# matter-labs/era-zkevm_test_harness

Measured on AMD Instinct MI355X. Metric: base-layer circuits/sec (2^20 rows); full-block synth wall-time 1/8 GPU, higher is better.
Workload: dtype u64 (Goldilocks, p = 2^64 - 2^32 + 1)

## Files before the change

era_zkevm_test_harness_amd/csrc/radix_sort.cuh:

```cuda
#pragma once
#include "zkw_ctx.h"

namespace zkw {

constexpr int RS_ROUNDS = 8, RS_WAVES = 4, RS_TILE = RS_WAVES * RS_ROUNDS * 64, RS_CHUNK = 16384;

template <class K>
static __device__ __forceinline__ unsigned rs_digit(K key, unsigned shift, unsigned mask) { return (unsigned)(key >> shift) & mask; }

template <class K>
static __device__ __forceinline__ void k_rs_hist(const VB& vb, const K* __restrict__ keys, size_t n, unsigned shift, unsigned mask, u32* __restrict__ hist, u32 n_tiles) {
    __shared__ u32 cnt[256];
    const int t = threadIdx.x;
    cnt[t] = 0;
    __syncthreads();
    const size_t base = (size_t)vb.x * RS_TILE;
#pragma unroll 4
    for (int r = 0; r < RS_TILE / 256; r++) {
        const size_t i = base + (size_t)r * 256 + t;
        if (i < n) atomicAdd(&cnt[rs_digit(keys[i], shift, mask)], 1u);
    }
    __syncthreads();
    hist[(size_t)t * n_tiles + vb.x] = cnt[t];
}

static __device__ __forceinline__ void k_rs_scan_a(const VB& vb, u32* __restrict__ hist, size_t n_entries, u32* __restrict__ chunk_tot) {
    __shared__ u32 s_wave[16];
    const int t = threadIdx.x, lane = t & 63, wave = t >> 6;
    const size_t base = (size_t)vb.x * RS_CHUNK + (size_t)t * 16;
    u32 v[16], sum = 0;
#pragma unroll
    for (int k = 0; k < 16; k++) {
        v[k] = base + k < n_entries ? hist[base + k] : 0;
        sum += v[k];
    }
    u32 incl = sum;
#pragma unroll
    for (int off = 1; off < 64; off <<= 1) {
        const u32 y = __shfl_up(incl, off, 64);
        if (lane >= off) incl += y;
    }
    if (lane == 63) s_wave[wave] = incl;
    __syncthreads();
    u32 before = 0;
    for (int w = 0; w < wave; w++) before += s_wave[w];
    u32 run = before + incl - sum;
#pragma unroll
    for (int k = 0; k < 16; k++) {
        if (base + k < n_entries) hist[base + k] = run;
        run += v[k];
    }
    if (t == 1023) chunk_tot[vb.x] = before + incl;
}

static __device__ __forceinline__ void k_rs_scan_b(const VB& vb, u32* __restrict__ chunk_tot, u32 n_chunks) {
    __shared__ u32 s_wave[16];
    __shared__ u32 carry;
    const int t = threadIdx.x, lane = t & 63, wave = t >> 6;
    if (t == 0) carry = 0;
    __syncthreads();
    for (u32 base = 0; base < n_chunks; base += 1024) {
        const u32 i = base + t;
        const u32 v = i < n_chunks ? chunk_tot[i] : 0;
        u32 incl = v;
#pragma unroll
        for (int off = 1; off < 64; off <<= 1) {
            const u32 y = __shfl_up(incl, off, 64);
            if (lane >= off) incl += y;
        }
        if (lane == 63) s_wave[wave] = incl;
        __syncthreads();
        u32 before = carry;
        for (int w = 0; w < wave; w++) before += s_wave[w];
        if (i < n_chunks) chunk_tot[i] = before + incl - v;
        __syncthreads();
        if (t == 1023) carry = before + incl;
        __syncthreads();
    }
}

template <class K>
static __device__ __forceinline__ void k_rs_scatter(const VB& vb, const K* __restrict__ kin, const u32* __restrict__ vin, size_t n, unsigned shift, unsigned mask,
                                    const u32* __restrict__ hist, const u32* __restrict__ chunk_off, u32 n_tiles, K* __restrict__ kout, u32* __restrict__ vout) {
    __shared__ K s_key[RS_TILE];
    __shared__ u32 s_val[RS_TILE];
    __shared__ u32 wcnt[RS_WAVES][256];
    __shared__ u32 s_first[256];
    __shared__ u32 s_gbase[256];
    __shared__ u32 s_wsum[RS_WAVES];
    const int t = threadIdx.x, lane = t & 63, wave = t >> 6;
#pragma unroll
    for (int w = 0; w < RS_WAVES; w++) wcnt[w][t] = 0;
    __syncthreads();
    const size_t tile0 = (size_t)vb.x * RS_TILE, base = tile0 + (size_t)wave * (RS_ROUNDS * 64) + lane;
    K key[RS_ROUNDS];
    u32 val[RS_ROUNDS];
    unsigned long long same[RS_ROUNDS];
#pragma unroll
    for (int r = 0; r < RS_ROUNDS; r++) {
        const size_t i = base + (size_t)r * 64;
        key[r] = i < n ? kin[i] : (K)0;
        val[r] = i < n ? vin[i] : 0u;
    }
#pragma unroll
    for (int r = 0; r < RS_ROUNDS; r++) {
        const size_t i = base + (size_t)r * 64;
        const bool ok = i < n;
        const unsigned d = rs_digit(key[r], shift, mask);
        unsigned long long m = __ballot(ok);
#pragma unroll
        for (int b = 0; b < 8; b++) {
            const unsigned long long bal = __ballot((d >> b) & 1);
            m &= ((d >> b) & 1) ? bal : ~bal;
        }
        same[r] = ok ? m : 0ull;
        if (ok && (m & ((1ull << lane) - 1)) == 0) wcnt[wave][d] += (u32)__popcll(m);
        __builtin_amdgcn_wave_barrier();
    }
    __syncthreads();
    {
        u32 c[RS_WAVES], total = 0;
#pragma unroll
        for (int w = 0; w < RS_WAVES; w++) { c[w] = wcnt[w][t]; total += c[w]; }
        u32 incl = total;
#pragma unroll
        for (int off = 1; off < 64; off <<= 1) {
            const u32 y = __shfl_up(incl, off, 64);
            if (lane >= off) incl += y;
        }
        if (lane == 63) s_wsum[wave] = incl;
        __syncthreads();
        u32 first = incl - total;
        for (int w = 0; w < wave; w++) first += s_wsum[w];
        s_first[t] = first;
        const size_t e = (size_t)t * n_tiles + vb.x;
        s_gbase[t] = hist[e] + chunk_off[e / RS_CHUNK] - first;
        u32 at = first;
#pragma unroll
        for (int w = 0; w < RS_WAVES; w++) { wcnt[w][t] = at; at += c[w]; }
    }
    __syncthreads();
#pragma unroll
    for (int r = 0; r < RS_ROUNDS; r++) {
        const unsigned long long m = same[r];
        if (m) {
            const unsigned d = rs_digit(key[r], shift, mask);
            const u32 at = wcnt[wave][d] + (u32)__popcll(m & ((1ull << lane) - 1));
            s_key[at] = key[r];
            s_val[at] = val[r];
        }
        __builtin_amdgcn_wave_barrier();
        if (m && (m & ((1ull << lane) - 1)) == 0) wcnt[wave][rs_digit(key[r], shift, mask)] += (u32)__popcll(m);
        __builtin_amdgcn_wave_barrier();
    }
    __syncthreads();
    const u32 in_tile = (u32)(n - tile0 < (size_t)RS_TILE ? n - tile0 : (size_t)RS_TILE);
#pragma unroll 4
    for (u32 p = t; p < in_tile; p += 256) {
        const K k = s_key[p];
        const u32 at = s_gbase[rs_digit(k, shift, mask)] + p;
        kout[at] = k;
        vout[at] = s_val[p];
    }
}

static inline size_t rs_tiles(size_t n) { return (n + RS_TILE - 1) / RS_TILE; }
static inline size_t radix_temp_bytes(size_t n) {
    const size_t entries = 256 * rs_tiles(n), chunks = (entries + RS_CHUNK - 1) / RS_CHUNK;
    return ((n * 8 + 255) & ~(size_t)255) + ((n * 4 + 255) & ~(size_t)255) + entries * 4 + chunks * 4 + 1024;
}

template <class K>
static int radix_sort_pairs(zkw_ctx* ctx, void* tmp, size_t tmp_bytes, const K* kin, K* kout, const u32* vin, u32* vout, size_t n, unsigned end_bit) {
    if (n == 0) return ZKW_OK;
    if (n >= (1ull << 32)) return fail(ZKW_ERR_INVALID, "radix_sort_pairs: more than 2^32 - 1 pairs");
    if (tmp_bytes < radix_temp_bytes(n)) return fail(ZKW_ERR_INVALID, "radix_sort_pairs: temporary storage too small");
    if (end_bit == 0) end_bit = 1;
    const unsigned passes = (end_bit + 7) / 8;
    const u32 n_tiles = (u32)rs_tiles(n);
    const size_t entries = (size_t)256 * n_tiles;
    const u32 n_chunks = (u32)((entries + RS_CHUNK - 1) / RS_CHUNK);
    char* p = static_cast<char*>(tmp);
    K* tk = reinterpret_cast<K*>(p);
    u32* tv = reinterpret_cast<u32*>(p + ((n * 8 + 255) & ~(size_t)255));
    u32* hist = reinterpret_cast<u32*>(p + ((n * 8 + 255) & ~(size_t)255) + ((n * 4 + 255) & ~(size_t)255));
    u32* chunk = hist + entries;
    const K* src_k = kin;
    const u32* src_v = vin;
    for (unsigned pass = 0; pass < passes; pass++) {
        const bool to_out = ((passes - pass) & 1) == 1;
        K* dst_k = to_out ? kout : tk;
        u32* dst_v = to_out ? vout : tv;
        const unsigned shift = 8 * pass, bits = std::min(8u, end_bit - shift), mask = (1u << bits) - 1;
        ZKW_LAUNCH_T(ctx, (k_rs_hist<K>), "k_rs_hist", n_tiles, 256, src_k, n, shift, mask, hist, n_tiles);
        ZKW_LAUNCH(ctx, k_rs_scan_a, n_chunks, 1024, hist, entries, chunk);
        ZKW_LAUNCH(ctx, k_rs_scan_b, 1, 1024, chunk, n_chunks);
        ZKW_LAUNCH_T(ctx, (k_rs_scatter<K>), "k_rs_scatter", n_tiles, 256, src_k, src_v, n, shift, mask, (const u32*)hist, (const u32*)chunk, n_tiles, dst_k, dst_v);
        src_k = dst_k;
        src_v = dst_v;
    }
    return ZKW_OK;
}

}
```

era_zkevm_test_harness_amd/csrc/ram_kernels.cuh:

```cuda
#pragma once
#include "../../include/zkw_types.h"
#include "poseidon2.cuh"

namespace zkw {
using gl::u32;
using gl::u64;

__device__ __forceinline__ void encode_mem_query(const zkw_mem_query& q, u64 out[8]) {
    const u32* v = q.value;
    out[0] = q.timestamp;
    out[1] = q.page;
    out[2] = (u64)q.index | ((u64)(q.rw_flag ? 1 : 0) << 32) | ((u64)(q.value_is_pointer ? 1 : 0) << 33);
    u64 b5 = v[5], b6 = v[6], b7 = v[7];
    out[3] = (u64)v[0] | ((b5 & 0xFFFFFF) << 32);
    out[4] = (u64)v[1] | ((b5 >> 24) << 32) | ((b6 & 0xFFFF) << 40);
    out[5] = (u64)v[2] | ((b6 >> 16) << 32) | ((b7 & 0xFF) << 48);
    out[6] = (u64)v[3] | ((b7 >> 8) << 32);
    out[7] = v[4];
}

static __device__ __forceinline__ void k_encode_mem(const VB& vb, const zkw_mem_query* __restrict__ q, size_t n,
                                                    u64* __restrict__ enc) {
    size_t i = (size_t)vb.x * blockDim.x + threadIdx.x;
    size_t stride = (size_t)vb.nx * blockDim.x;
    for (; i < n; i += stride) {
        const uint4* src = reinterpret_cast<const uint4*>(q + i);
        uint4 w0 = src[0], w1 = src[1], w2 = src[2];
        zkw_mem_query m;
        uint4* dst = reinterpret_cast<uint4*>(&m);
        dst[0] = w0; dst[1] = w1; dst[2] = w2;
        u64 e[8];
        encode_mem_query(m, e);
        ulonglong2* o = reinterpret_cast<ulonglong2*>(enc + 8 * i);
        o[0] = make_ulonglong2(e[0], e[1]); o[1] = make_ulonglong2(e[2], e[3]);
        o[2] = make_ulonglong2(e[4], e[5]); o[3] = make_ulonglong2(e[6], e[7]);
    }
}

struct ChainJob {
    const u64* enc;
    u64* tails;
    const u64* tail_in;
    u64 n;
    u64* caps;
    u64* marks;
    u64 period;
    const zkw_mem_query* q;
    const u32* perm;
};

struct RawQuery { uint4 a, b, c; };
__device__ __forceinline__ RawQuery load_raw_query(const zkw_mem_query* q) {
    const uint4* src = reinterpret_cast<const uint4*>(q);
    RawQuery r;
    r.a = src[0]; r.b = src[1]; r.c = src[2];
    return r;
}
__device__ __forceinline__ void encode_raw_query(const RawQuery& r, u64 e[8]) {
    zkw_mem_query m;
    uint4* dm = reinterpret_cast<uint4*>(&m);
    dm[0] = r.a; dm[1] = r.b; dm[2] = r.c;
    encode_mem_query(m, e);
}
__device__ __forceinline__ u64 pick8(const u64 e[8], int g) {
    u64 v = e[0];
#pragma unroll
    for (int k = 1; k < 8; k++) v = g == k ? e[k] : v;
    return v;
}


struct RowForm {
    static constexpr int LANES = 16, N = 1, R = 1;
    p2::Coop co;
    int g;
    __device__ __forceinline__ void init(int j) { g = j; co.init(j); }
    __device__ __forceinline__ bool reads_items() const { return g < 8; }
    __device__ __forceinline__ void load_tail(const u64* t, u64 x[N]) const { x[0] = (co.active && t) ? t[g] : 0; }
    __device__ __forceinline__ void load_rate(const u64* enc, u64 e[R]) const { e[0] = enc[g]; }
    __device__ __forceinline__ void pick_rate(const u64 ew[8], u64 e[R]) const { e[0] = pick8(ew, g); }
    __device__ __forceinline__ void absorb_permute(u64 x[N], const u64 e[R]) const { x[0] = co.permute(g < 8 ? e[0] : x[0]); }
    __device__ __forceinline__ void store_tail(u64* t, const u64 p[N]) const { if (co.active) t[g] = p[0]; }
    __device__ __forceinline__ void store_caps(u64* c, const u64 p[N]) const { if (g >= 8 && g < 12) c[g - 8] = p[0]; }
};

struct QuadForm {
    static constexpr int LANES = 4, N = 3, R = 2;
    p2::Coop4 co;
    int j;
    __device__ __forceinline__ void init(int j_) { j = j_; co.init(j_); }
    __device__ __forceinline__ bool reads_items() const { return true; }
    __device__ __forceinline__ void load_tail(const u64* t, u64 x[N]) const {
#pragma unroll
        for (int c = 0; c < 3; c++) x[c] = t ? t[4 * c + j] : 0;
    }
    __device__ __forceinline__ void load_rate(const u64* enc, u64 e[R]) const { e[0] = enc[j]; e[1] = enc[4 + j]; }
    __device__ __forceinline__ void pick_rate(const u64 ew[8], u64 e[R]) const { e[0] = pick8(ew, j); e[1] = pick8(ew, 4 + j); }
    __device__ __forceinline__ void absorb_permute(u64 x[N], const u64 e[R]) const { x[0] = e[0]; x[1] = e[1]; co.permute(x); }
    __device__ __forceinline__ void store_tail(u64* t, const u64 p[N]) const {
#pragma unroll
        for (int c = 0; c < 3; c++) t[4 * c + j] = p[c];
    }
    __device__ __forceinline__ void store_caps(u64* c, const u64 p[N]) const { c[j] = p[2]; }
};

struct PairForm {
    static constexpr int LANES = 2, N = 6, R = 4;
    p2::Coop2 co;
    int j;
    __device__ __forceinline__ void init(int j_) { j = j_; co.init(j_); }
    __device__ __forceinline__ bool reads_items() const { return true; }
    __device__ __forceinline__ void load_tail(const u64* t, u64 x[N]) const {
#pragma unroll
        for (int c = 0; c < 3; c++) {
            x[2 * c] = t ? t[4 * c + 2 * j] : 0;
            x[2 * c + 1] = t ? t[4 * c + 2 * j + 1] : 0;
        }
    }
    __device__ __forceinline__ void load_rate(const u64* enc, u64 e[R]) const {
        const ulonglong2 lo = *reinterpret_cast<const ulonglong2*>(enc + 2 * j), hi = *reinterpret_cast<const ulonglong2*>(enc + 4 + 2 * j);
        e[0] = lo.x; e[1] = lo.y; e[2] = hi.x; e[3] = hi.y;
    }
    __device__ __forceinline__ void pick_rate(const u64 ew[8], u64 e[R]) const {
        e[0] = j ? ew[2] : ew[0];
        e[1] = j ? ew[3] : ew[1];
        e[2] = j ? ew[6] : ew[4];
        e[3] = j ? ew[7] : ew[5];
    }
    __device__ __forceinline__ void absorb_permute(u64 x[N], const u64 e[R]) const {
#pragma unroll
        for (int k = 0; k < 4; k++) x[k] = e[k];
        co.permute(x);
    }
    __device__ __forceinline__ void store_tail(u64* t, const u64 p[N]) const {
#pragma unroll
        for (int c = 0; c < 3; c++) *reinterpret_cast<ulonglong2*>(t + 4 * c + 2 * j) = make_ulonglong2(p[2 * c], p[2 * c + 1]);
    }
    __device__ __forceinline__ void store_caps(u64* c, const u64 p[N]) const { *reinterpret_cast<ulonglong2*>(c + 2 * j) = make_ulonglong2(p[4], p[5]); }
};

struct LaneForm {
    static constexpr int LANES = 1, N = 12, R = 8;
    __device__ __forceinline__ void init(int) {}
    __device__ __forceinline__ bool reads_items() const { return true; }
    __device__ __forceinline__ void load_tail(const u64* t, u64 x[N]) const {
#pragma unroll
        for (int k = 0; k < 12; k++) x[k] = t ? t[k] : 0;
    }
    __device__ __forceinline__ void load_rate(const u64* enc, u64 e[R]) const {
        const ulonglong2* src = reinterpret_cast<const ulonglong2*>(enc);
#pragma unroll
        for (int k = 0; k < 4; k++) { const ulonglong2 v = src[k]; e[2 * k] = v.x; e[2 * k + 1] = v.y; }
    }
    __device__ __forceinline__ void pick_rate(const u64 ew[8], u64 e[R]) const {
#pragma unroll
        for (int k = 0; k < 8; k++) e[k] = ew[k];
    }
    __device__ __forceinline__ void absorb_permute(u64 x[N], const u64 e[R]) const {
#pragma unroll
        for (int k = 0; k < 8; k++) x[k] = e[k];
        p2::permute(x);
    }
    __device__ __forceinline__ void store_tail(u64* t, const u64 p[N]) const {
        ulonglong2* d = reinterpret_cast<ulonglong2*>(t);
#pragma unroll
        for (int k = 0; k < 6; k++) d[k] = make_ulonglong2(p[2 * k], p[2 * k + 1]);
    }
    __device__ __forceinline__ void store_caps(u64* c, const u64 p[N]) const {
        ulonglong2* d = reinterpret_cast<ulonglong2*>(c);
        d[0] = make_ulonglong2(p[8], p[9]);
        d[1] = make_ulonglong2(p[10], p[11]);
    }
};

template <class Form, int WAVES>
static __device__ __forceinline__ void chain_body(const ChainJob* __restrict__ jobs, int n_jobs) {
    __builtin_amdgcn_s_setprio(3);
    const int chain = blockIdx.x * (64 * WAVES / Form::LANES) + threadIdx.x / Form::LANES;
    Form form;
    form.init(threadIdx.x % Form::LANES);
    ChainJob job;
    memset(&job, 0, sizeof job);
    if (chain < n_jobs) job = jobs[chain];
    u64 x[Form::N];
    form.load_tail(job.tail_in, x);
    const bool reads = form.reads_items();
    const bool from_q = job.enc == nullptr;
    u64 e_next[Form::R] = {};
    RawQuery rq_next;
    rq_next.a = rq_next.b = rq_next.c = make_uint4(0, 0, 0, 0);
    u64 at_next = 0;
    if (reads && job.n > 0) {
        if (from_q) rq_next = load_raw_query(job.q + (job.perm ? job.perm[0] : 0)); else form.load_rate(job.enc, e_next);
    }
    if (reads && from_q && job.n > 1) at_next = job.perm ? job.perm[1] : 1;
    u64 next_mark = job.marks ? job.period : ~0ull, mark_idx = 0;
    u64 pend[Form::N] = {}, pend_i = 0;
    bool have_pend = false, pend_mark = false;
    auto flush = [&]() {
        if (!have_pend) return;
        if (job.tails) form.store_tail(job.tails + 12 * pend_i, pend);
        if (job.caps) form.store_caps(job.caps + 4 * pend_i, pend);
        if (pend_mark) form.store_tail(job.marks + 12 * mark_idx++, pend);
        have_pend = false;
    };
    for (u64 i = 0; __any(i < job.n); i++) {
        const bool live = i < job.n;
        u64 e[Form::R];
        if (from_q) {
            u64 ew[8];
            encode_raw_query(rq_next, ew);
            form.pick_rate(ew, e);
        } else {
#pragma unroll
            for (int k = 0; k < Form::R; k++) e[k] = e_next[k];
        }
        flush();
        if (reads && i + 1 < job.n) {
            if (from_q) {
                rq_next = load_raw_query(job.q + at_next);
                if (i + 2 < job.n) at_next = job.perm ? job.perm[i + 2] : i + 2;
            } else {
                form.load_rate(job.enc + 8 * (i + 1), e_next);
            }
        }
        form.absorb_permute(x, e);
        if (live) {
#pragma unroll
            for (int k = 0; k < Form::N; k++) pend[k] = gl::canon(x[k]);
            pend_i = i;
            have_pend = true;
            pend_mark = job.marks && (i + 1 == next_mark || i + 1 == job.n);
            if (pend_mark) next_mark += job.period;
        }
    }
    flush();
}
static __global__ __launch_bounds__(64) void k_chain_full(const ChainJob* __restrict__ jobs, int n_jobs) { chain_body<RowForm, 1>(jobs, n_jobs); }
static __global__ __launch_bounds__(256) void k_chain_full_x4(const ChainJob* __restrict__ jobs, int n_jobs) { chain_body<RowForm, 4>(jobs, n_jobs); }
static __global__ __launch_bounds__(64) void k_chain_full_q4(const ChainJob* __restrict__ jobs, int n_jobs) { chain_body<QuadForm, 1>(jobs, n_jobs); }
static __global__ __launch_bounds__(256) void k_chain_full_q4x4(const ChainJob* __restrict__ jobs, int n_jobs) { chain_body<QuadForm, 4>(jobs, n_jobs); }
static __global__ __launch_bounds__(64) void k_chain_full_p2(const ChainJob* __restrict__ jobs, int n_jobs) { chain_body<PairForm, 1>(jobs, n_jobs); }
static __global__ __launch_bounds__(64) void k_chain_full_lane(const ChainJob* __restrict__ jobs, int n_jobs) { chain_body<LaneForm, 1>(jobs, n_jobs); }

struct FsJob {
    const u64* tail_u;
    const u64* tail_s;
    u32 len_u, len_s;
    u64* out;
};

static __device__ __forceinline__ void k_fs_challenges(const VB& vb, const FsJob* __restrict__ jobs, int n_jobs, int state_w, int n_chal) {
    int j = vb.x * blockDim.x + threadIdx.x;
    if (j >= n_jobs) return;
    const FsJob job = jobs[j];
    const int m = 2 * state_w + 2;
    auto elem = [&](int e) -> u64 {
        if (e >= m) return 0;
        if (e < state_w) return job.tail_u[e];
        if (e == state_w) return job.len_u;
        if (e < 2 * state_w + 1) return job.tail_s[e - state_w - 1];
        return job.len_s;
    };
    u64 s[12];
#pragma unroll
    for (int i = 0; i < 12; i++) s[i] = 0;
    s[11] = (u64)m;
    for (int i = 0; i < m; i += 8) {
#pragma unroll
        for (int k = 0; k < 8; k++) s[k] = elem(i + k);
        p2::permute(s);
    }
    int can_take = 8;
    for (int rep = 0; rep < 2; rep++) {
        job.out[rep * n_chal] = 1;
        for (int k = 1; k < n_chal; k++) {
            if (can_take == 0) { p2::permute(s); can_take = 8; }
            u64 v = 0;
#pragma unroll
            for (int q = 0; q < 8; q++) v = (q == 8 - can_take) ? s[q] : v;
            job.out[rep * n_chal + k] = gl::canon(v);
            can_take--;
        }
    }
}

constexpr int GP_BLOCK = 256;
constexpr int GP_SLABS = 4;
constexpr int GP_TILE = GP_BLOCK * GP_SLABS;

struct GpSeg {
    const u64* rows;
    u64* z;
    const u64* chal;
    u64 n;
    u32 first_tile;
    u32 n_tiles;
    const zkw_mem_query* mem_q;
    const u32* perm;
};
struct GpTile {
    u32 seg;
    u32 tile;
};

__device__ __forceinline__ u64 wave_scan_mul(u64 v, int lane) {
#pragma unroll
    for (int d = 1; d < 64; d <<= 1) {
        u64 o = __shfl_up(v, d, 64);
        if (lane >= d) v = gl::mul(v, o);
    }
    return v;
}

template <int W, int REPS>
static __device__ __forceinline__ void k_gp_local(const VB& vb, const GpSeg* __restrict__ segs,
                                                       const GpTile* __restrict__ tiles,
                                                       u64* __restrict__ tile_aggr ) {
    __shared__ u64 sh_ch[REPS][W + 1];
    __shared__ u64 sh_wave[REPS][GP_BLOCK / 64];
    const GpTile t = tiles[vb.x];
    const GpSeg seg = segs[t.seg];
    const int tid = threadIdx.x, lane = tid & 63, wave = tid >> 6;
    for (int k = tid; k < REPS * (W + 1); k += GP_BLOCK) sh_ch[k / (W + 1)][k % (W + 1)] = seg.chal[k];
    __syncthreads();
    u64 carry[REPS];
#pragma unroll
    for (int r = 0; r < REPS; r++) carry[r] = 1;
    const u64 base = (u64)t.tile * GP_TILE;
    for (int slab = 0; slab < GP_SLABS; slab++) {
        const u64 row = base + (u64)slab * GP_BLOCK + tid;
        const bool live = row < seg.n;
        u64 term[REPS];
#pragma unroll
        for (int r = 0; r < REPS; r++) term[r] = 1;
        if (live) {
            u64 e[W];
            if (W == 8 && seg.rows == nullptr) {
                u64 e8[8];
                encode_raw_query(load_raw_query(seg.mem_q + (seg.perm ? seg.perm[row] : row)), e8);
#pragma unroll
                for (int k = 0; k < (W < 8 ? W : 8); k++) e[k] = e8[k];
            } else {
                const ulonglong2* src = reinterpret_cast<const ulonglong2*>(seg.rows + row * W);
#pragma unroll
                for (int k = 0; k < W / 2; k++) { ulonglong2 w = src[k]; e[2 * k] = w.x; e[2 * k + 1] = w.y; }
            }
#pragma unroll
            for (int r = 0; r < REPS; r++) {
                u64 acc = sh_ch[r][W];
#pragma unroll
                for (int k = 0; k < W; k++) acc = gl::add(acc, gl::mul(e[k], sh_ch[r][k]));
                term[r] = acc;
            }
        }
#pragma unroll
        for (int r = 0; r < REPS; r++) {
            u64 v = wave_scan_mul(term[r], lane);
            if (lane == 63) sh_wave[r][wave] = v;
            __syncthreads();
            u64 pre = carry[r];
            for (int w = 0; w < wave; w++) pre = gl::mul(pre, sh_wave[r][w]);
            v = gl::mul(v, pre);
            if (live) seg.z[(u64)r * seg.n + row] = v;
            u64 tot = carry[r];
            for (int w = 0; w < GP_BLOCK / 64; w++) tot = gl::mul(tot, sh_wave[r][w]);
            carry[r] = tot;
            __syncthreads();
        }
    }
    if (tid == 0) {
#pragma unroll
        for (int r = 0; r < REPS; r++) tile_aggr[(u64)vb.x * REPS + r] = carry[r];
    }
}

template <int REPS>
static __device__ __forceinline__ void k_gp_tiles(const VB& vb, const GpSeg* __restrict__ segs, int n_segs, u64* __restrict__ tile_aggr) {
    int j = vb.x * blockDim.x + threadIdx.x;
    if (j >= n_segs * REPS) return;
    const GpSeg seg = segs[j / REPS];
    const int r = j % REPS;
    u64 acc = 1;
    for (u32 t = 0; t < seg.n_tiles; t++) {
        u64* p = tile_aggr + (u64)(seg.first_tile + t) * REPS + r;
        u64 v = *p;
        *p = acc;
        acc = gl::mul(acc, v);
    }
}

template <int REPS>
static __device__ __forceinline__ void k_gp_apply(const VB& vb, const GpSeg* __restrict__ segs,
                                                       const GpTile* __restrict__ tiles,
                                                       const u64* __restrict__ tile_prefix) {
    const GpTile t = tiles[vb.x];
    const GpSeg seg = segs[t.seg];
    const u64 base = (u64)t.tile * GP_TILE;
#pragma unroll
    for (int r = 0; r < REPS; r++) {
        const u64 pre = tile_prefix[(u64)vb.x * REPS + r];
        u64* z = seg.z + (u64)r * seg.n;
        for (int slab = 0; slab < GP_SLABS; slab++) {
            const u64 row = base + (u64)slab * GP_BLOCK + threadIdx.x;
            if (row < seg.n) z[row] = gl::canon(gl::mul(z[row], pre));
        }
    }
}

static __device__ __forceinline__ void k_ram_sort_keys(const VB& vb, const zkw_mem_query* __restrict__ q, size_t n, u32* __restrict__ ts,
                                u64* __restrict__ cell, u32* __restrict__ iota, const u64* __restrict__ seg_off,
                                int n_segs) {
    size_t i = (size_t)vb.x * blockDim.x + threadIdx.x;
    if (i >= n) return;
    ts[i] = q[i].timestamp;
    cell[i] = ((u64)q[i].page << 32) | q[i].index;
    iota[i] = (u32)i;
    (void)seg_off; (void)n_segs;
}

static __device__ __forceinline__ void k_gather_u32_by_u32(const VB& vb, const u32* __restrict__ src, const u32* __restrict__ idx, size_t n,
                                    u32* __restrict__ dst) {
    size_t i = (size_t)vb.x * blockDim.x + threadIdx.x;
    if (i < n) dst[i] = src[idx[i]];
}

static __device__ __forceinline__ void k_gather_u64_by_u32(const VB& vb, const u64* __restrict__ src, const u32* __restrict__ idx, size_t n,
                                    u64* __restrict__ dst) {
    size_t i = (size_t)vb.x * blockDim.x + threadIdx.x;
    if (i < n) dst[i] = src[idx[i]];
}

static __device__ __forceinline__ void k_gather_encode(const VB& vb, const zkw_mem_query* __restrict__ q,
                                                       const u32* __restrict__ perm, size_t n,
                                                       zkw_mem_query* __restrict__ sorted_q,
                                                       u64* __restrict__ sorted_enc) {
    size_t i = (size_t)vb.x * blockDim.x + threadIdx.x;
    if (i >= n) return;
    const uint4* src = reinterpret_cast<const uint4*>(q + perm[i]);
    uint4 w0 = src[0], w1 = src[1], w2 = src[2];
    uint4* dq = reinterpret_cast<uint4*>(sorted_q + i);
    dq[0] = w0; dq[1] = w1; dq[2] = w2;
    zkw_mem_query m;
    uint4* dm = reinterpret_cast<uint4*>(&m);
    dm[0] = w0; dm[1] = w1; dm[2] = w2;
    if (!sorted_enc) return;
    u64 e[8];
    encode_mem_query(m, e);
    ulonglong2* o = reinterpret_cast<ulonglong2*>(sorted_enc + 8 * i);
    o[0] = make_ulonglong2(e[0], e[1]); o[1] = make_ulonglong2(e[2], e[3]);
    o[2] = make_ulonglong2(e[4], e[5]); o[3] = make_ulonglong2(e[6], e[7]);
}

struct RamBlock {
    const zkw_mem_query* sorted_q;
    const u32* sorted_perm;
    const u64* u_marks;
    const u64* s_marks;
    const u64* lhs_z;
    const u64* rhs_z;
    zkw_ram_instance* instances;
    u32* nondet_prefix;
    u64* gp_ckpt;
    u32* nd_prefix;
    u64 n;
    u32 capacity;
    u32 num_nondet_heap_queries;
};

__device__ __forceinline__ void copy12(u64* dst, const u64* src) {
    for (int k = 0; k < 12; k++) dst[k] = src[k];
}

static __device__ __forceinline__ void k_ram_count_nondet(const VB& vb, const RamBlock* __restrict__ blocks) {
    const RamBlock b = blocks[vb.y];
    const u64 n_inst = (b.n + b.capacity - 1) / b.capacity;
    const u32 n_tiles = (b.capacity + 255) / 256;
    __shared__ u32 sh[2][2][4];
    for (u64 inst = vb.x; inst < n_inst; inst += vb.nx) {
        const u64 lo = inst * b.capacity, hi = lo + b.capacity < b.n ? lo + b.capacity : b.n;
        u32 cnt = 0, before = 0;
        for (u32 t = 0; t < n_tiles; t++) {
            const u64 i = lo + 256 * (u64)t + threadIdx.x;
            bool f = false, fc = false;
            if (i < hi) {
                const zkw_mem_query* q = b.sorted_q + b.sorted_perm[i];
                f = q->rw_flag && q->timestamp == 0 && q->page == ZKW_BOOTLOADER_HEAP_PAGE;
                fc = f && !q->value_is_pointer;
            }
            const u32 c = __popcll(__ballot(f)), cc = __popcll(__ballot(fc));
            if ((threadIdx.x & 63) == 0) { sh[t & 1][0][threadIdx.x >> 6] = c; sh[t & 1][1][threadIdx.x >> 6] = cc; }
            __syncthreads();
            if (threadIdx.x == 0) {
                const u32* s0 = sh[t & 1][0];
                const u32* s1 = sh[t & 1][1];
                b.nd_prefix[inst * n_tiles + t] = before;
                cnt += s0[0] + s0[1] + s0[2] + s0[3];
                before += s1[0] + s1[1] + s1[2] + s1[3];
            }
        }
        if (threadIdx.x == 0) b.nondet_prefix[inst] = cnt;
        __syncthreads();
    }
}

static __device__ __forceinline__ void k_ram_instances(const VB& vb, const RamBlock* __restrict__ blocks) {
    const RamBlock b = blocks[vb.y];
    const u64 n_inst = (b.n + b.capacity - 1) / b.capacity;
    const u64 idx = (u64)vb.x * blockDim.x + threadIdx.x;
    if (idx >= n_inst) return;
    const u64 n = b.n, lo = idx * b.capacity, hi = lo + b.capacity < n ? lo + b.capacity : n;
    zkw_ram_instance& w = b.instances[idx];
    memset(&w, 0, sizeof w);
    w.start_flag = idx == 0;
    w.completion_flag = idx == n_inst - 1;
    w.first_item = lo;
    w.num_items = hi - lo;
    const u64* u_final = b.u_marks + 12 * (n_inst - 1);
    const u64* s_final = b.s_marks + 12 * (n_inst - 1);
    copy12(w.unsorted_queue_initial_state.tail, u_final);
    w.unsorted_queue_initial_state.length = (u32)n;
    copy12(w.sorted_queue_initial_state.tail, s_final);
    w.sorted_queue_initial_state.length = (u32)n;
    w.non_deterministic_bootloader_memory_snapshot_length = b.num_nondet_heap_queries;

    u32 nondet_before = 0;
    for (u64 k = 0; k < idx; k++) nondet_before += b.nondet_prefix[k];

    auto fill = [&](zkw_ram_fsm& f, u64 end , u32 nondet) {
        const u64 l = end - 1;
        for (int r = 0; r < 2; r++) { f.lhs_accumulator[r] = b.lhs_z[r * n + l]; f.rhs_accumulator[r] = b.rhs_z[r * n + l]; }
        copy12(f.current_unsorted_queue_state.head, b.u_marks + 12 * (l / b.capacity));
        copy12(f.current_unsorted_queue_state.tail, u_final);
        f.current_unsorted_queue_state.length = (u32)(n - end);
        copy12(f.current_sorted_queue_state.head, b.s_marks + 12 * (l / b.capacity));
        copy12(f.current_sorted_queue_state.tail, s_final);
        f.current_sorted_queue_state.length = (u32)(n - end);
        const zkw_mem_query* q = b.sorted_q + b.sorted_perm[l];
        f.previous_sorting_key[0] = q->timestamp; f.previous_sorting_key[1] = q->index; f.previous_sorting_key[2] = q->page;
        f.previous_full_key[0] = q->index; f.previous_full_key[1] = q->page;
        for (int k = 0; k < 8; k++) f.previous_value[k] = q->value[k];
        f.previous_is_ptr = q->value_is_pointer ? 1 : 0;
        f.num_nondeterministic_writes = nondet;
    };
    if (idx == 0) {
        for (int r = 0; r < 2; r++) { w.hidden_fsm_input.lhs_accumulator[r] = 1; w.hidden_fsm_input.rhs_accumulator[r] = 1; }
    } else {
        fill(w.hidden_fsm_input, lo, nondet_before);
    }
    fill(w.hidden_fsm_output, hi, nondet_before + b.nondet_prefix[idx]);
    if ((hi - lo) % b.capacity != 0) {
        zkw_ram_fsm& f = w.hidden_fsm_output;
        for (int k = 0; k < 3; k++) f.previous_sorting_key[k] = 0;
        for (int k = 0; k < 2; k++) f.previous_full_key[k] = 0;
        for (int k = 0; k < 8; k++) f.previous_value[k] = 0;
        f.previous_is_ptr = 0;
    }
}

static __device__ __forceinline__ void k_ram_gp_ckpt(const VB& vb, const RamBlock* __restrict__ blocks) {
    const RamBlock b = blocks[vb.y];
    const u64 n_inst = (b.n + b.capacity - 1) / b.capacity, groups = (b.capacity + 63) / 64;
    const u64 j = (u64)vb.x * blockDim.x + threadIdx.x;
    if (j >= n_inst * groups) return;
    const u64 idx = j / groups, g = j % groups;
    const zkw_ram_instance& in = b.instances[idx];
    const u64 first = in.first_item, m = in.num_items;
    u64* out = b.gp_ckpt + 4 * j;
    for (int r = 0; r < 2; r++) {
        const u64 at = (u64)r * b.n + first + (64 * g - 1 < m ? 64 * g - 1 : m - 1);
        out[r] = g == 0 ? in.hidden_fsm_input.lhs_accumulator[r] : b.lhs_z[at];
        out[2 + r] = g == 0 ? in.hidden_fsm_input.rhs_accumulator[r] : b.rhs_z[at];
    }
}

static __device__ __forceinline__ void k_tails_expand(const VB& vb, const u64* __restrict__ enc, const u64* __restrict__ caps,
                                                     const u64* __restrict__ offsets, int n_queues, size_t n,
                                                     u64* __restrict__ tails) {
    const size_t i = (size_t)vb.x * blockDim.x + threadIdx.x;
    if (i >= n) return;
    int lo = 0, hi = n_queues;
    while (hi - lo > 1) {
        const int mid = (lo + hi) >> 1;
        if (offsets[mid] <= i) lo = mid; else hi = mid;
    }
    u64 s[12];
#pragma unroll
    for (int k = 0; k < 8; k++) s[k] = enc[8 * i + k];
    const bool first = offsets[lo] == i;
#pragma unroll
    for (int k = 0; k < 4; k++) s[8 + k] = first ? 0 : caps[4 * (i - 1) + k];
    p2::permute(s);
#pragma unroll
    for (int k = 0; k < 12; k++) tails[12 * i + k] = gl::canon(s[k]);
}

}
```

era_zkevm_test_harness_amd/csrc/zkw_api.hip:

```cpp
#include "zkw_ctx.h"
#include "circuit_check_host.h"
#include "closed_forms_host.h"
#include "callstack_kernels.cuh"
#include "vm_kernels.cuh"
#include "radix_sort.cuh"

static thread_local std::string g_last_error;

#undef fail
int zkw_fail(int code, const char* fmt, ...) {
    char buf[512];
    va_list ap;
    va_start(ap, fmt);
    vsnprintf(buf, sizeof buf, fmt, ap);
    va_end(ap);
    g_last_error = buf;
    return code;
}

#define fail zkw_fail

struct AllocCache {
    static constexpr size_t SMALL_MAX = size_t(256) << 20;
    static constexpr int MAX_DEV = 16;
    std::mutex mu;
    std::map<const void*, std::pair<int, size_t>> live[2];
    std::map<size_t, std::vector<void*>> idle[2][MAX_DEV];
    const bool enabled = [] { const char* e = getenv("ZKW_ALLOC_CACHE"); return !(e && e[0] == '0'); }();

    static size_t size_class(size_t b) {
        if (b <= 4096) return 4096;
        if (b > SMALL_MAX) return (b + ((size_t(2) << 20) - 1)) & ~((size_t(2) << 20) - 1);
        int top = 63 - __builtin_clzll(b);
        const size_t step = size_t(1) << (top - 3);
        return (b + step - 1) & ~(step - 1);
    }
    static hipError_t raw_alloc(int host, void** p, size_t bytes) {
        return host ? hipHostMalloc(p, bytes, hipHostMallocDefault) : hipMalloc(p, bytes);
    }
    hipError_t alloc(int host, void** p, size_t bytes) {
        int dev = 0;
        if (!enabled || hipGetDevice(&dev) != hipSuccess || dev >= MAX_DEV) return raw_alloc(host, p, bytes);
        const size_t cls = size_class(bytes);
        {
            std::lock_guard<std::mutex> g(mu);
            auto it = idle[host][dev].find(cls);
            if (it != idle[host][dev].end() && !it->second.empty()) {
                *p = it->second.back();
                it->second.pop_back();
                live[host][*p] = {dev, cls};
                return hipSuccess;
            }
        }
        hipError_t e = raw_alloc(host, p, cls);
        if (e != hipSuccess) {
            (void)hipGetLastError();
            static std::atomic<int> n_trims{0};
            if (n_trims.fetch_add(1) < 8)
                fprintf(stderr, "[zkw] out of %s memory at a request of %zu bytes: the allocation cache is emptied and the request retried (expect a stall)\n", host ? "pinned host" : "device", cls);
            trim();
            e = raw_alloc(host, p, cls);
        }
        if (e == hipSuccess) {
            std::lock_guard<std::mutex> g(mu);
            live[host][*p] = {dev, cls};
        }
        return e;
    }
    void release(int host, void* p) {
        if (!p) return;
        {
            std::lock_guard<std::mutex> g(mu);
            auto it = live[host].find(p);
            if (it != live[host].end()) {
                idle[host][it->second.first][it->second.second].push_back(p);
                live[host].erase(it);
                return;
            }
        }
        if (host) (void)hipHostFree(p); else (void)hipFree(p);
    }
    void trim() {
        std::vector<void*> d, h;
        {
            std::lock_guard<std::mutex> g(mu);
            for (int dev = 0; dev < MAX_DEV; ++dev) {
                for (auto& kv : idle[0][dev]) { d.insert(d.end(), kv.second.begin(), kv.second.end()); kv.second.clear(); }
                for (auto& kv : idle[1][dev]) { h.insert(h.end(), kv.second.begin(), kv.second.end()); kv.second.clear(); }
            }
        }
        for (void* q : d) (void)hipFree(q);
        for (void* q : h) (void)hipHostFree(q);
    }
};
static AllocCache& alloc_cache() {
    static AllocCache* c = new AllocCache();
    return *c;
}
hipError_t zkw_cache_alloc(int pinned_host, void** p, size_t bytes) { return alloc_cache().alloc(pinned_host ? 1 : 0, p, bytes); }
void zkw_cache_release(int pinned_host, void* p) { alloc_cache().release(pinned_host ? 1 : 0, p); }


struct StreamPool {
    std::mutex mu;
    std::vector<hipStream_t> idle[AllocCache::MAX_DEV];
    hipError_t acquire(hipStream_t* s) {
        int dev = 0;
        if (alloc_cache().enabled && hipGetDevice(&dev) == hipSuccess && dev < AllocCache::MAX_DEV) {
            std::lock_guard<std::mutex> g(mu);
            if (!idle[dev].empty()) {
                *s = idle[dev].back();
                idle[dev].pop_back();
                return hipSuccess;
            }
        }
        return hipStreamCreateWithFlags(s, hipStreamNonBlocking);
    }
    void release(hipStream_t s) {
        if (!s) return;
        int dev = 0;
        if (alloc_cache().enabled && hipGetDevice(&dev) == hipSuccess && dev < AllocCache::MAX_DEV) {
            std::lock_guard<std::mutex> g(mu);
            idle[dev].push_back(s);
            return;
        }
        (void)hipStreamDestroy(s);
    }
    void trim() {
        std::vector<hipStream_t> all;
        {
            std::lock_guard<std::mutex> g(mu);
            for (auto& v : idle) { all.insert(all.end(), v.begin(), v.end()); v.clear(); }
        }
        for (hipStream_t s : all) (void)hipStreamDestroy(s);
    }
};
static StreamPool& stream_pool() {
    static StreamPool* p = new StreamPool();
    return *p;
}

hipError_t zkw_pool_stream_acquire(hipStream_t* s) { return stream_pool().acquire(s); }
void zkw_pool_stream_release(hipStream_t s) { stream_pool().release(s); }

extern "C" void zkw_trim_caches(void) {
    alloc_cache().trim();
    stream_pool().trim();
}

extern "C" const char* zkw_last_error(void) { return g_last_error.c_str(); }
extern "C" const char* zkw_version(void) { return "zkw 0.2 (gfx950)"; }

extern "C" zkw_ctx* zkw_create(int device_id) {
    int count = 0;
    hipError_t e = hipGetDeviceCount(&count);
    if (e != hipSuccess || count == 0) {
        fail(ZKW_ERR_NO_DEVICE, "no HIP device available (%s); libzkw has no CPU fallback",
             e == hipSuccess ? "device count is 0" : hipGetErrorString(e));
        return nullptr;
    }
    if (device_id < 0 || device_id >= count) {
        fail(ZKW_ERR_INVALID, "device_id %d out of range [0, %d)", device_id, count);
        return nullptr;
    }
    if (hipSetDevice(device_id) != hipSuccess) {
        fail(ZKW_ERR_HIP, "hipSetDevice(%d) failed", device_id);
        return nullptr;
    }
    hipDeviceProp_t prop;
    if (hipGetDeviceProperties(&prop, device_id) == hipSuccess) {
        if (strncmp(prop.gcnArchName, "gfx950", 6) != 0) {
            fail(ZKW_ERR_NO_DEVICE, "device %d is %s; libzkw kernels are built for gfx950 only", device_id,
                 prop.gcnArchName);
            return nullptr;
        }
    }
    zkw_ctx* ctx = new zkw_ctx();
    ctx->device = device_id;
    if (stream_pool().acquire(&ctx->own_stream) != hipSuccess) {
        fail(ZKW_ERR_HIP, "hipStreamCreate failed");
        delete ctx;
        return nullptr;
    }
    ctx->stream = ctx->own_stream;
    return ctx;
}

static void ctx_destroy_now(zkw_ctx* ctx) {
    (void)hipSetDevice(ctx->device);
    (void)hipStreamSynchronize(ctx->stream);
    for (auto& kv : ctx->pool)
        if (kv.second.p) dev_free(kv.second.p);
    for (auto& sp : ctx->spans) { (void)hipEventDestroy(sp.a); (void)hipEventDestroy(sp.b); }
    for (auto e : ctx->free_events) (void)hipEventDestroy(e);
    for (auto& kv : ctx->stages) {
        if (kv.second.p) pin_free(kv.second.p);
        if (kv.second.ev) (void)hipEventDestroy(kv.second.ev);
    }
    for (void* q : ctx->retired_dev) dev_free(q);
    for (void* q : ctx->retired_host) pin_free(q);
    if (ctx->pinned_rb) pin_free(ctx->pinned_rb);
    if (ctx->chain_ev_a) (void)hipEventDestroy(ctx->chain_ev_a);
    if (ctx->chain_ev_b) (void)hipEventDestroy(ctx->chain_ev_b);
    if (ctx->side_stream) {
        (void)hipStreamSynchronize(ctx->side_stream);
        stream_pool().release(ctx->side_stream);
    }
    if (ctx->side_ev_fork) {
        (void)hipEventDestroy(ctx->side_ev_fork);
        (void)hipEventDestroy(ctx->side_ev_join);
    }
    if (ctx->own_stream) {
        (void)hipStreamSynchronize(ctx->own_stream);
        stream_pool().release(ctx->own_stream);
    }
    delete ctx;
}
void ctx_retain(zkw_ctx* ctx) { ctx->children.fetch_add(1); }
int zkw_ctx_device(const zkw_ctx* ctx) { return ctx->device; }
void* zkw_ctx_stream(const zkw_ctx* ctx) { return ctx->stream; }
void zkw_ctx_retain(zkw_ctx* ctx) { ctx_retain(ctx); }
void zkw_ctx_release(zkw_ctx* ctx) { ctx_release(ctx); }
static void ctx_try_destroy(zkw_ctx* ctx) {
    bool expected = false;
    if (ctx->destroying.compare_exchange_strong(expected, true)) ctx_destroy_now(ctx);
}
void ctx_release(zkw_ctx* ctx) {
    if (ctx->children.fetch_sub(1) == 1 && ctx->destroy_requested.load()) ctx_try_destroy(ctx);
}

extern "C" void zkw_destroy(zkw_ctx* ctx) {
    if (!ctx) return;
    if (ctx->children.load() > 0) {
        (void)hipSetDevice(ctx->device);
        (void)hipStreamSynchronize(ctx->stream);
    }
    ctx->destroy_requested.store(true);
    if (ctx->children.load() == 0) ctx_try_destroy(ctx);
}

extern "C" int zkw_set_stream(zkw_ctx* ctx, void* s) {
    if (!ctx) return fail(ZKW_ERR_INVALID, "null context");
    HIP_TRY(hipStreamSynchronize(ctx->stream));
    ctx->stream = (s == ZKW_STREAM_OWN) ? ctx->own_stream : static_cast<hipStream_t>(s);
    return ZKW_OK;
}

extern "C" int zkw_buffer_alloc(zkw_ctx* ctx, int pinned_host, size_t bytes, void** out) {
    if (!ctx || !out) return fail(ZKW_ERR_INVALID, "zkw_buffer_alloc: null argument");
    HIP_TRY(hipSetDevice(ctx->device));
    *out = nullptr;
    hipError_t e = pinned_host ? pin_malloc(out, bytes ? bytes : 1) : dev_malloc(out, bytes ? bytes : 1);
    if (e != hipSuccess) {
        (void)hipGetLastError();
        return fail(ZKW_ERR_OOM, "zkw_buffer_alloc: %zu bytes of %s memory: %s", bytes, pinned_host ? "pinned host" : "device", hipGetErrorString(e));
    }
    return ZKW_OK;
}
extern "C" void zkw_buffer_free(int pinned_host, void* p) {
    if (pinned_host) pin_free(p); else dev_free(p);
}
extern "C" int zkw_stream_acquire(zkw_ctx* ctx, void** stream) {
    if (!ctx || !stream) return fail(ZKW_ERR_INVALID, "zkw_stream_acquire: null argument");
    HIP_TRY(hipSetDevice(ctx->device));
    hipStream_t s = nullptr;
    HIP_TRY(stream_pool().acquire(&s));
    *stream = s;
    return ZKW_OK;
}
extern "C" void zkw_stream_release(zkw_ctx* ctx, void* stream) {
    if (!ctx || !stream) return;
    (void)hipSetDevice(ctx->device);
    (void)hipStreamSynchronize(static_cast<hipStream_t>(stream));
    stream_pool().release(static_cast<hipStream_t>(stream));
}

extern "C" int zkw_set_chain_stream(zkw_ctx* ctx, void* s) {
    if (!ctx) return fail(ZKW_ERR_INVALID, "null context");
    HIP_TRY(hipStreamSynchronize(ctx->stream));
    if (s && !(ctx->chain_ev_a && ctx->chain_ev_b)) {
        hipEvent_t a = nullptr, b = nullptr;
        HIP_TRY(hipEventCreateWithFlags(&a, hipEventDisableTiming));
        hipError_t e = hipEventCreateWithFlags(&b, hipEventDisableTiming);
        if (e != hipSuccess) {
            (void)hipEventDestroy(a);
            return fail(ZKW_ERR_HIP, "hipEventCreate failed: %s", hipGetErrorString(e));
        }
        if (ctx->chain_ev_a) (void)hipEventDestroy(ctx->chain_ev_a);
        if (ctx->chain_ev_b) (void)hipEventDestroy(ctx->chain_ev_b);
        ctx->chain_ev_a = a;
        ctx->chain_ev_b = b;
    }
    ctx->chain_stream = static_cast<hipStream_t>(s);
    return ZKW_OK;
}

extern "C" int zkw_set_pointer_mode(zkw_ctx* ctx, int mode) {
    if (!ctx || (mode != ZKW_PTR_HOST && mode != ZKW_PTR_DEVICE)) return fail(ZKW_ERR_INVALID, "bad pointer mode");
    ctx->ptr_mode = mode;
    return ZKW_OK;
}

extern "C" int zkw_set_chain_form(zkw_ctx* ctx, int lanes_per_state) {
    if (!ctx || (lanes_per_state != 0 && lanes_per_state != 1 && lanes_per_state != 2 && lanes_per_state != 4 && lanes_per_state != 16))
        return fail(ZKW_ERR_INVALID, "chain form must be 0 (auto), 1, 2, 4 or 16");
    ctx->chain_form = lanes_per_state;
    return ZKW_OK;
}

extern "C" int zkw_set_netlist_fill_form(zkw_ctx* ctx, int form) {
    if (!ctx || (form != 0 && form != 1)) return fail(ZKW_ERR_INVALID, "netlist fill form must be 0 (a wave per cycle) or 1 (a lane per cycle)");
    ctx->netlist_fill_form = form;
    return ZKW_OK;
}

extern "C" int zkw_synchronize(zkw_ctx* ctx) {
    if (!ctx) return fail(ZKW_ERR_INVALID, "null context");
    if (ctx->batched()) return zkw_batch_sync(ctx->batch);
    HIP_TRY(ctx->sync_stream());
    return ZKW_OK;
}

zkw_ctx* zkw_ctx_create_in_batch(int device_id, zkw_batch* b) {
    zkw_ctx* ctx = new zkw_ctx();
    ctx->device = device_id;
    ctx->batch = b;
    ctx->stream = zkw_batch_stream(b);
    ctx->ptr_mode = ZKW_PTR_DEVICE;
    return ctx;
}
size_t zkw_ctx_scratch_bytes(const zkw_ctx* ctx) {
    size_t b = 0;
    for (auto& kv : ctx->pool) b += kv.second.cap;
    for (void* q : ctx->retired_dev) { (void)q; }
    return b;
}
void zkw_ctx_scratch_mark(const zkw_ctx* ctx, std::vector<std::string>* names) {
    names->clear();
    for (auto& kv : ctx->pool) names->push_back(kv.first);
}
void zkw_ctx_scratch_release_since(zkw_ctx* ctx, const std::vector<std::string>& names) {
    for (auto it = ctx->pool.begin(); it != ctx->pool.end();) {
        if (std::find(names.begin(), names.end(), it->first) == names.end()) {
            if (it->second.p) dev_free(it->second.p);
            it = ctx->pool.erase(it);
        } else {
            ++it;
        }
    }
}
void zkw_cache_stats(size_t* live_bytes, size_t* idle_bytes) {
    AllocCache& c = alloc_cache();
    std::lock_guard<std::mutex> g(c.mu);
    size_t l = 0, i = 0;
    for (auto& kv : c.live[0]) l += kv.second.second;
    for (int d = 0; d < AllocCache::MAX_DEV; d++)
        for (auto& kv : c.idle[0][d]) i += kv.first * kv.second.size();
    *live_bytes = l;
    *idle_bytes = i;
}
int zkw_copy_device(zkw_ctx* ctx, void* dst, const void* src, size_t bytes) {
    if (!ctx) return fail(ZKW_ERR_INVALID, "null context");
    if (bytes) HIP_TRY(ctx->copy_async(dst, src, bytes, hipMemcpyDeviceToDevice));
    return ZKW_OK;
}
void* zkw_device_shared_stream(int device_id) {
    static std::mutex mu;
    static std::map<int, hipStream_t>& m = *new std::map<int, hipStream_t>();
    std::lock_guard<std::mutex> g(mu);
    auto it = m.find(device_id);
    if (it != m.end()) return it->second;
    hipStream_t s = nullptr;
    if (hipSetDevice(device_id) != hipSuccess || hipStreamCreateWithFlags(&s, hipStreamNonBlocking) != hipSuccess) return nullptr;
    m[device_id] = s;
    return s;
}
void zkw_ctx_enter_batch(zkw_ctx* ctx, zkw_batch* b) {
    ctx->batch = b;
    ctx->stream = zkw_batch_stream(b);
}
zkw_batch* zkw_ctx_swap_batch(zkw_ctx* ctx, zkw_batch* b) {
    zkw_batch* old = ctx->batch;
    ctx->batch = b;
    return old;
}
void zkw_ctx_leave_batch(zkw_ctx* ctx, void* stream) {
    ctx->batch = nullptr;
    ctx->stream = static_cast<hipStream_t>(stream);
}

extern "C" int zkw_profile_enable(zkw_ctx* ctx, int on) {
    if (!ctx) return fail(ZKW_ERR_INVALID, "null context");
    ZKW_TRY(ctx->prof_collect());
    ctx->profiling = on != 0;
    return ZKW_OK;
}

extern "C" int zkw_profile_reset(zkw_ctx* ctx) {
    if (!ctx) return fail(ZKW_ERR_INVALID, "null context");
    ZKW_TRY(ctx->prof_collect());
    ctx->prof_totals.clear();
    return ZKW_OK;
}

extern "C" int zkw_profile_get(zkw_ctx* ctx, const char* kernel, double* total_ms, uint64_t* launches) {
    if (!ctx || !kernel) return fail(ZKW_ERR_INVALID, "null argument");
    ZKW_TRY(ctx->prof_collect());
    auto it = ctx->prof_totals.find(kernel);
    if (total_ms) *total_ms = it == ctx->prof_totals.end() ? 0.0 : it->second.first;
    if (launches) *launches = it == ctx->prof_totals.end() ? 0 : it->second.second;
    return ZKW_OK;
}

extern "C" int zkw_profile_names(zkw_ctx* ctx, char* buf, size_t buf_bytes) {
    if (!ctx || !buf || !buf_bytes) return fail(ZKW_ERR_INVALID, "null argument");
    ZKW_TRY(ctx->prof_collect());
    std::string all;
    for (auto& kv : ctx->prof_totals) { if (!all.empty()) all += ","; all += kv.first; }
    if (all.size() + 1 > buf_bytes) return fail(ZKW_ERR_INVALID, "buffer too small: need %zu bytes", all.size() + 1);
    memcpy(buf, all.c_str(), all.size() + 1);
    return ZKW_OK;
}

static int one_workgroup_per_cu_lds(const void* func, int slot ) {
    static std::atomic<int> lds_of[4][64];
    int dev = 0;
    if (hipGetDevice(&dev) != hipSuccess || dev < 0 || dev >= 64) return -1;
    int lds = lds_of[slot][dev].load();
    if (lds == 0) {
        int per_cu = 0;
        if (hipDeviceGetAttribute(&per_cu, hipDeviceAttributeMaxSharedMemoryPerMultiprocessor, dev) != hipSuccess || per_cu <= 0) per_cu = 160 * 1024;
        const int want = (per_cu / 2 + 4096) & ~1023;
        lds = hipFuncSetAttribute(func, hipFuncAttributeMaxDynamicSharedMemorySize, want) == hipSuccess ? want : -1;
        if (lds < 0) (void)hipGetLastError();
        lds_of[slot][dev].store(lds);
    }
    return lds;
}
static const char* launch_chain(int form, bool allow_wg4, hipStream_t st, const ChainJob* d_jobs, int n_jobs) {
    static const bool wg4_env = [] { const char* e = getenv("ZKW_CHAIN_WG4"); return !(e && e[0] == '0'); }();
    const bool wg4 = allow_wg4 && wg4_env;
    const unsigned per_wave = 64 / form, waves = (n_jobs + per_wave - 1) / per_wave;
    if (form == 4) {
        const int lds = wg4 && n_jobs > 64 && n_jobs <= 256 * 64 ? one_workgroup_per_cu_lds(reinterpret_cast<const void*>(&k_chain_full_q4x4), 0) : -1;
        if (lds > 0) { hipLaunchKernelGGL(k_chain_full_q4x4, dim3((waves + 3) / 4), dim3(256), (size_t)lds, st, d_jobs, n_jobs); return "k_chain_full_q4x4"; }
        hipLaunchKernelGGL(k_chain_full_q4, dim3(waves), dim3(64), 0, st, d_jobs, n_jobs);
        return "k_chain_full_q4";
    }
    if (form == 16) {
        const int lds = wg4 && n_jobs > 4 && n_jobs <= 256 * 16 ? one_workgroup_per_cu_lds(reinterpret_cast<const void*>(&k_chain_full_x4), 1) : -1;
        if (lds > 0) { hipLaunchKernelGGL(k_chain_full_x4, dim3((waves + 3) / 4), dim3(256), (size_t)lds, st, d_jobs, n_jobs); return "k_chain_full_x4"; }
        hipLaunchKernelGGL(k_chain_full, dim3(waves), dim3(64), 0, st, d_jobs, n_jobs);
        return "k_chain_full";
    }
    if (form == 2) { hipLaunchKernelGGL(k_chain_full_p2, dim3(waves), dim3(64), 0, st, d_jobs, n_jobs); return "k_chain_full_p2"; }
    hipLaunchKernelGGL(k_chain_full_lane, dim3(waves), dim3(64), 0, st, d_jobs, n_jobs);
    return "k_chain_full_lane";
}
static void launch_chain_log_rows(hipStream_t st, const LogChainJob* d_jobs, int n_jobs) {
    static const bool wg4 = [] { const char* e = getenv("ZKW_CHAIN_WG4"); const char* l = getenv("ZKW_CHAIN_LOG_WG4"); return !(e && e[0] == '0') && !(l && l[0] == '0'); }();
    const int lds = wg4 && n_jobs > 4 && n_jobs <= 256 * 16 ? one_workgroup_per_cu_lds(reinterpret_cast<const void*>(&k_chain_log_x4), 2) : -1;
    if (lds > 0) hipLaunchKernelGGL(k_chain_log_x4, dim3((n_jobs + 15) / 16), dim3(256), (size_t)lds, st, d_jobs, n_jobs);
    else hipLaunchKernelGGL(k_chain_log, dim3((n_jobs + 3) / 4), dim3(64), 0, st, d_jobs, n_jobs);
}

int zkw_launch_chain_full(hipStream_t st, const ChainJob* d_jobs, int n_jobs) {
    launch_chain(n_jobs >= 4096 ? 4 : 16, true, st, d_jobs, n_jobs);
    return ZKW_OK;
}
int zkw_launch_chain_log(hipStream_t st, const LogChainJob* d_jobs, int n_jobs) {
    for (int at = 0; at < n_jobs; at += 4096) launch_chain_log_rows(st, d_jobs + at, std::min(4096, n_jobs - at));
    return ZKW_OK;
}

struct ChainService {
    struct Batch {
        std::vector<ChainJob> full;
        std::vector<LogChainJob> log;
        int waiters = 0;
        bool done[2] = {false, false};
        int rc = ZKW_OK;
        std::string err;
        int key = 0;
        std::chrono::steady_clock::time_point open_since, last_arrival;
    };
    int device = 0;
    std::mutex mu;
    std::condition_variable cv_work, cv_done;
    std::map<int, std::shared_ptr<Batch>> open;
    int expected = 0;
    std::vector<std::thread> workers;
    bool stop = false;

    int n_workers = 8;
    long quiet_us = 4000, max_us = 40000, quiet_long_us = 100000;
    explicit ChainService(int dev) : device(dev) {
        if (const char* e = getenv("ZKW_CHAIN_WORKERS")) n_workers = std::max(1, std::min(32, atoi(e)));
        if (const char* e = getenv("ZKW_CHAIN_WINDOW_US")) { quiet_us = std::max(50L, atol(e)); max_us = 10 * quiet_us; }
        if (const char* e = getenv("ZKW_CHAIN_LONG_WINDOW_US")) quiet_long_us = std::max(50L, atol(e));
        for (int i = 0; i < n_workers; i++) workers.emplace_back([this] { run(); });
    }
    ~ChainService() {
        { std::lock_guard<std::mutex> g(mu); stop = true; }
        cv_work.notify_all();
        for (auto& t : workers) t.join();
    }
    void expect(int delta) {
        { std::lock_guard<std::mutex> g(mu); expected = std::max(0, expected + delta); }
        cv_work.notify_all();
    }
    bool ready(const Batch& b, std::chrono::steady_clock::time_point now) const {
        if (b.key != 0 && expected > 1) {
            if (b.waiters >= expected) return true;
            return now - b.last_arrival >= std::chrono::microseconds(quiet_long_us) || now - b.open_since >= std::chrono::microseconds(10 * quiet_long_us);
        }
        return now - b.last_arrival >= std::chrono::microseconds(quiet_us) || now - b.open_since >= std::chrono::microseconds(max_us);
    }
    int submit(const std::vector<ChainJob>* full, const std::vector<LogChainJob>* log, std::string* err, int key) {
        std::shared_ptr<Batch> b;
        {
            std::unique_lock<std::mutex> lk(mu);
            std::shared_ptr<Batch>& slot = open[key];
            const auto now = std::chrono::steady_clock::now();
            if (!slot) { slot = std::make_shared<Batch>(); slot->key = key; slot->open_since = now; }
            b = slot;
            if (full) b->full.insert(b->full.end(), full->begin(), full->end());
            if (log) b->log.insert(b->log.end(), log->begin(), log->end());
            b->waiters++;
            b->last_arrival = now;
            cv_work.notify_one();
            const int kind = full ? 0 : 1;
            cv_done.wait(lk, [&] { return b->done[kind]; });
            const int rc = b->rc;
            if (rc != ZKW_OK && err) *err = b->err;
            return rc;
        }
    }
    void skip(int key) {
        if (key == 0) return;
        {
            std::lock_guard<std::mutex> g(mu);
            if (expected <= 1) return;
            std::shared_ptr<Batch>& slot = open[key];
            const auto now = std::chrono::steady_clock::now();
            if (!slot) { slot = std::make_shared<Batch>(); slot->key = key; slot->open_since = now; }
            slot->waiters++;
            slot->last_arrival = now;
        }
        cv_work.notify_one();
    }
    void run() {
        (void)hipSetDevice(device);
        hipStream_t st = nullptr, st_log = nullptr;
        int lo = 0, hi = 0;
        (void)hipDeviceGetStreamPriorityRange(&lo, &hi);
        if (hipStreamCreateWithPriority(&st, hipStreamNonBlocking, hi) != hipSuccess) st = nullptr;
        void* pin = nullptr;
        void* dev = nullptr;
        size_t cap = 0;
        for (;;) {
            std::shared_ptr<Batch> b;
            {
                std::unique_lock<std::mutex> lk(mu);
                for (;;) {
                    if (stop) break;
                    const auto now = std::chrono::steady_clock::now();
                    auto best = open.end();
                    for (auto it = open.begin(); it != open.end(); ++it)
                        if (it->second && ready(*it->second, now) && (best == open.end() || it->second->open_since < best->second->open_since)) best = it;
                    if (best != open.end()) { b = best->second; open.erase(best); break; }
                    if (open.empty()) cv_work.wait(lk, [&] { return stop || !open.empty(); });
                    else cv_work.wait_for(lk, std::chrono::microseconds(200));
                }
                if (stop) break;
            }
            int rc = ZKW_OK;
            std::string err;
            auto fail_hip = [&](hipError_t e, const char* what) { if (e != hipSuccess && rc == ZKW_OK) { rc = ZKW_ERR_HIP; err = std::string(what) + ": " + hipGetErrorString(e); } };
            static const bool log_batches = getenv("ZKW_CHAIN_LOG") != nullptr;
            const auto t_launch = std::chrono::steady_clock::now();
            size_t longest = 0;
            if (log_batches) for (const ChainJob& j : b->full) longest = std::max(longest, (size_t)j.n);
            const size_t bytes = b->full.size() * sizeof(ChainJob) + b->log.size() * sizeof(LogChainJob) + 256;
            const bool mixed = !b->full.empty() && !b->log.empty();
            if (mixed && !st_log && hipStreamCreateWithPriority(&st_log, hipStreamNonBlocking, hi) != hipSuccess) st_log = nullptr;
            hipStream_t sl = mixed ? st_log : st;
            if (!st || !sl) { rc = ZKW_ERR_HIP; err = "chain service: no stream"; }
            const bool nothing = b->full.empty() && b->log.empty();
            if (rc == ZKW_OK && !nothing && cap < bytes) {
                const size_t want = bytes * 2;
                void *np = nullptr, *nd = nullptr;
                fail_hip(pin_malloc(&np, want), "hipHostMalloc");
                if (rc == ZKW_OK) fail_hip(dev_malloc(&nd, want), "hipMalloc");
                if (rc == ZKW_OK) {
                    if (pin) pin_free(pin);
                    if (dev) dev_free(dev);
                    pin = np; dev = nd; cap = want;
                } else if (np) {
                    pin_free(np);
                }
            }
            if (rc == ZKW_OK && !nothing) {
                char* hp = static_cast<char*>(pin);
                char* dp = static_cast<char*>(dev);
                const size_t off_log = (b->full.size() * sizeof(ChainJob) + 127) & ~(size_t)127;
                if (!b->full.empty()) memcpy(hp, b->full.data(), b->full.size() * sizeof(ChainJob));
                if (!b->log.empty()) memcpy(hp + off_log, b->log.data(), b->log.size() * sizeof(LogChainJob));
                fail_hip(hipMemcpyAsync(dp, hp, off_log + b->log.size() * sizeof(LogChainJob), hipMemcpyHostToDevice, st), "job upload");
                fail_hip(hipStreamSynchronize(st), "job upload");
                const int nf = (int)b->full.size(), nl = (int)b->log.size();
                if (rc == ZKW_OK && nl) launch_chain_log_rows(sl, reinterpret_cast<const LogChainJob*>(dp + off_log), nl);
                if (rc == ZKW_OK && nf) launch_chain(nf >= 4096 ? 4 : 16, true, st, reinterpret_cast<const ChainJob*>(dp), nf);
                fail_hip(hipGetLastError(), "chain launch");
                fail_hip(hipStreamSynchronize(sl), "chain batch (log queues)");
                {
                    std::lock_guard<std::mutex> g(mu);
                    if (rc != ZKW_OK) { b->rc = rc; b->err = err; }
                    b->done[1] = true;
                }
                cv_done.notify_all();
                fail_hip(hipStreamSynchronize(st), "chain batch");
            }
            {
                std::lock_guard<std::mutex> g(mu);
                if (rc != ZKW_OK) { b->rc = rc; b->err = err; }
                b->done[0] = b->done[1] = true;
            }
            cv_done.notify_all();
            if (log_batches) {
                static const auto t_zero = std::chrono::steady_clock::now();
                const auto us = [&](std::chrono::steady_clock::time_point t) { return (long)std::chrono::duration_cast<std::chrono::microseconds>(t - t_zero).count(); };
                fprintf(stderr, "[zkw chain] batch of %d waiters: %zu full-width chains (longest %zu items), %zu log chains; left at %ld us, done at %ld us\n", b->waiters, b->full.size(), longest,
                        b->log.size(), us(t_launch), us(std::chrono::steady_clock::now()));
            }
        }
        if (pin) pin_free(pin);
        if (dev) dev_free(dev);
        if (st) (void)hipStreamDestroy(st);
        if (st_log) (void)hipStreamDestroy(st_log);
    }
};
static std::mutex g_chain_services_mu;
static std::map<int, ChainService*>& g_chain_services = *new std::map<int, ChainService*>();
static ChainService* chain_service_of(int device) {
    std::lock_guard<std::mutex> g(g_chain_services_mu);
    ChainService*& p = g_chain_services[device];
    if (!p) p = new ChainService(device);
    return p;
}

extern "C" int zkw_chain_service_expect(int device_id, int delta) {
    if (device_id < 0) return fail(ZKW_ERR_INVALID, "zkw_chain_service_expect: bad device");
    chain_service_of(device_id)->expect(delta);
    return ZKW_OK;
}
extern "C" int zkw_set_chain_tag(zkw_ctx* ctx, int tag) {
    if (!ctx || tag < 0 || tag > 1000) return fail(ZKW_ERR_INVALID, "zkw_set_chain_tag: bad argument");
    ctx->chain_tag = tag;
    ctx->chain_seq = 0;
    return ZKW_OK;
}

extern "C" int zkw_set_chain_service(zkw_ctx* ctx, int on) {
    if (!ctx) return fail(ZKW_ERR_INVALID, "null context");
    ctx->chain_service = on != 0;
    if (on) (void)chain_service_of(ctx->device);
    return ZKW_OK;
}

static int chain_service_run(zkw_ctx* ctx, const std::vector<ChainJob>* full, const std::vector<LogChainJob>* log, const char* name, int key) {
    HIP_TRY(hipStreamSynchronize(ctx->stream));
    const auto t0 = std::chrono::steady_clock::now();
    std::string err;
    const int rc = chain_service_of(ctx->device)->submit(full, log, &err, key);
    if (ctx->profiling) {
        auto& t = ctx->prof_totals[std::string(name) + "(service)"];
        t.first += std::chrono::duration<double, std::milli>(std::chrono::steady_clock::now() - t0).count();
        t.second += 1;
    }
    if (rc != ZKW_OK) return fail(rc, "chain service: %s", err.c_str());
    return ZKW_OK;
}


int dev_encode(zkw_ctx* ctx, const zkw_mem_query* q, size_t n, u64* enc) {
    if (n == 0) return ZKW_OK;
    unsigned grid = blocks_for(n, 256);
    if (grid > 256 * 16) grid = 256 * 16;
    { Prof _p(ctx, "k_encode_mem"); ZKW_LAUNCH(ctx, k_encode_mem, grid, 256, q, n, enc); }
    return launch_check("k_encode_mem");
}

int dev_chains(zkw_ctx* ctx, const std::vector<ChainJob>& jobs) {
    if (ctx->batched()) return jobs.empty() ? ZKW_OK : zkw_batch_chains(ctx->batch, jobs.data(), jobs.size(), nullptr, 0);
    const int key = ctx->chain_service ? ctx->next_chain_key() : 0;
    if (jobs.empty()) { if (ctx->chain_service) chain_service_of(ctx->device)->skip(key); return ZKW_OK; }
    u64 longest = 0;
    for (const ChainJob& j : jobs) longest = std::max<u64>(longest, j.n);
    if (ctx->chain_service && longest > 64) return chain_service_run(ctx, &jobs, nullptr, "k_chain_full", key);
    if (ctx->chain_service) chain_service_of(ctx->device)->skip(key);
    ChainJob* d_jobs = nullptr;
    ZKW_TRY(ctx->upload("chain_jobs", jobs, &d_jobs));
    int n_jobs = (int)jobs.size();
    const int form = ctx->chain_form ? ctx->chain_form : (n_jobs >= 4096 ? 4 : 16);
    hipStream_t st = ctx->stream;
    if (ctx->chain_stream) {
        HIP_TRY(hipEventRecord(ctx->chain_ev_a, ctx->stream));
        HIP_TRY(hipStreamWaitEvent(ctx->chain_stream, ctx->chain_ev_a, 0));
        st = ctx->chain_stream;
    }
    const char* name = form == 16 ? "k_chain_full" : form == 4 ? "k_chain_full_q4" : form == 2 ? "k_chain_full_p2" : "k_chain_full_lane";
    const char* launched;
    {
        Prof _p(ctx, name);
        launched = launch_chain(form, form != 16, st, d_jobs, n_jobs);
        if (ctx->chain_stream) {
            HIP_TRY(hipEventRecord(ctx->chain_ev_b, ctx->chain_stream));
            HIP_TRY(hipStreamWaitEvent(ctx->stream, ctx->chain_ev_b, 0));
        }
    }
    return launch_check(launched);
}

int dev_fs(zkw_ctx* ctx, const std::vector<FsJob>& jobs, int state_w, int n_chal) {
    if (jobs.empty()) return ZKW_OK;
    FsJob* d_jobs = nullptr;
    ZKW_TRY(ctx->upload("fs_jobs", jobs, &d_jobs));
    int n = (int)jobs.size();
    { Prof _p(ctx, "k_fs_challenges"); ZKW_LAUNCH(ctx, k_fs_challenges, (n + 63) / 64, 64, d_jobs, n, state_w, n_chal); }
    return launch_check("k_fs_challenges");
}

template <int W, int REPS>
static int gp_launch(zkw_ctx* ctx, const GpSeg* d_segs, int n_segs, const GpTile* d_tiles, unsigned n_tiles,
                     u64* d_aggr) {
    { Prof _p(ctx, "k_gp_local"); ZKW_LAUNCH_T(ctx, (k_gp_local<W, REPS>), "k_gp_local", n_tiles, GP_BLOCK, d_segs, d_tiles, d_aggr); }
    ZKW_TRY(launch_check("k_gp_local"));
    { Prof _p(ctx, "k_gp_tiles"); ZKW_LAUNCH_T(ctx, (k_gp_tiles<REPS>), "k_gp_tiles", (n_segs * REPS + 63) / 64, 64, d_segs, n_segs, d_aggr); }
    ZKW_TRY(launch_check("k_gp_tiles"));
    { Prof _p(ctx, "k_gp_apply"); ZKW_LAUNCH_T(ctx, (k_gp_apply<REPS>), "k_gp_apply", n_tiles, GP_BLOCK, d_segs, d_tiles, d_aggr); }
    return launch_check("k_gp_apply");
}

int dev_grand_products(zkw_ctx* ctx, std::vector<GpSeg>& segs, int width, int n_reps) {
    std::vector<GpTile> tiles;
    for (size_t s = 0; s < segs.size(); s++) {
        segs[s].first_tile = (u32)tiles.size();
        segs[s].n_tiles = (u32)((segs[s].n + GP_TILE - 1) / GP_TILE);
        for (u32 t = 0; t < segs[s].n_tiles; t++) tiles.push_back(GpTile{(u32)s, t});
    }
    if (tiles.empty()) return ZKW_OK;
    GpSeg* d_segs = nullptr;
    GpTile* d_tiles = nullptr;
    u64* d_aggr = nullptr;
    ZKW_TRY(ctx->upload("gp_segs", segs, &d_segs));
    ZKW_TRY(ctx->upload("gp_tiles", tiles, &d_tiles));
    ZKW_TRY(ctx->scratch_t<u64>("gp_aggr", tiles.size() * 2, &d_aggr));
    const int n_segs = (int)segs.size();
    const unsigned n_tiles = (unsigned)tiles.size();
    if (width == 8 && n_reps == 2) return gp_launch<8, 2>(ctx, d_segs, n_segs, d_tiles, n_tiles, d_aggr);
    if (width == 8 && n_reps == 1) return gp_launch<8, 1>(ctx, d_segs, n_segs, d_tiles, n_tiles, d_aggr);
    if (width == 20 && n_reps == 2) return gp_launch<20, 2>(ctx, d_segs, n_segs, d_tiles, n_tiles, d_aggr);
    if (width == 20 && n_reps == 1) return gp_launch<20, 1>(ctx, d_segs, n_segs, d_tiles, n_tiles, d_aggr);
    return fail(ZKW_ERR_INVALID, "grand product: unsupported width %d / repetitions %d", width, n_reps);
}

extern "C" int zkw_encode_memory_queries(zkw_ctx* ctx, const zkw_mem_query* q, size_t n, uint64_t* enc) {
    if (!ctx || (n && (!q || !enc))) return fail(ZKW_ERR_INVALID, "zkw_encode_memory_queries: null argument");
    HIP_TRY(hipSetDevice(ctx->device));
    const zkw_mem_query* d_q = nullptr;
    u64* d_enc = nullptr;
    ZKW_TRY(ctx->in("enc_q", q, n, &d_q));
    ZKW_TRY(ctx->out("enc_out", enc, n * 8, &d_enc));
    ZKW_TRY(dev_encode(ctx, d_q, n, d_enc));
    ZKW_TRY(ctx->finish_out(enc, d_enc, n * 8));
    return ctx->sync_if_host();
}

extern "C" int zkw_queue_push_chain_full_batch(zkw_ctx* ctx, const uint64_t* enc, const uint64_t* offsets,
                                               size_t n_queues, const uint64_t* tails_in, uint64_t* tails) {
    if (!ctx || !offsets) return fail(ZKW_ERR_INVALID, "zkw_queue_push_chain_full_batch: null argument");
    HIP_TRY(hipSetDevice(ctx->device));
    for (size_t k = 0; k < n_queues; k++)
        if (offsets[k + 1] < offsets[k]) return fail(ZKW_ERR_INVALID, "offsets must be non-decreasing");
    const size_t total = n_queues ? offsets[n_queues] - offsets[0] : 0;
    if (total && (!enc || !tails)) return fail(ZKW_ERR_INVALID, "null enc/tails");
    const size_t base = n_queues ? offsets[0] : 0;
    const u64* d_enc = nullptr;
    const u64* d_tin = nullptr;
    u64* d_tails = nullptr;
    ZKW_TRY(ctx->in("chain_enc", enc + base * 8, total * 8, &d_enc));
    if (tails_in) ZKW_TRY(ctx->in("chain_tin", tails_in, n_queues * 12, &d_tin));
    ZKW_TRY(ctx->out("chain_tails", tails + base * 12, total * 12, &d_tails));
    std::vector<ChainJob> jobs(n_queues);
    for (size_t k = 0; k < n_queues; k++) {
        size_t lo = offsets[k] - base;
        jobs[k].enc = d_enc + lo * 8;
        jobs[k].tails = d_tails + lo * 12;
        jobs[k].tail_in = d_tin ? d_tin + 12 * k : nullptr;
        jobs[k].n = offsets[k + 1] - offsets[k];
    }
    ZKW_TRY(dev_chains(ctx, jobs));
    ZKW_TRY(ctx->finish_out(tails + base * 12, d_tails, total * 12));
    return ctx->sync_if_host();
}

extern "C" int zkw_queue_push_chain_full(zkw_ctx* ctx, const uint64_t* enc, size_t n, const uint64_t tail_in[12],
                                         uint64_t* tails) {
    uint64_t offsets[2] = {0, n};
    return zkw_queue_push_chain_full_batch(ctx, enc, offsets, 1, tail_in, tails);
}

extern "C" int zkw_fs_challenges(zkw_ctx* ctx, const uint64_t* tail_u, uint32_t len_u, const uint64_t* tail_s,
                                 uint32_t len_s, int state_w, int n_chal, uint64_t* out) {
    if (!ctx || !tail_u || !tail_s || !out) return fail(ZKW_ERR_INVALID, "zkw_fs_challenges: null argument");
    if ((state_w != 4 && state_w != 12) || n_chal < 1 || n_chal > 64)
        return fail(ZKW_ERR_INVALID, "zkw_fs_challenges: state_w must be 4 or 12, 1 <= n_chal <= 64");
    HIP_TRY(hipSetDevice(ctx->device));
    const u64 *d_u = nullptr, *d_s = nullptr;
    u64* d_out = nullptr;
    ZKW_TRY(ctx->in("fs_u", tail_u, (size_t)state_w, &d_u));
    ZKW_TRY(ctx->in("fs_s", tail_s, (size_t)state_w, &d_s));
    ZKW_TRY(ctx->out("fs_out", out, (size_t)2 * n_chal, &d_out));
    std::vector<FsJob> jobs(1);
    jobs[0] = FsJob{d_u, d_s, len_u, len_s, d_out};
    ZKW_TRY(dev_fs(ctx, jobs, state_w, n_chal));
    ZKW_TRY(ctx->finish_out(out, d_out, (size_t)2 * n_chal));
    return ctx->sync_if_host();
}

extern "C" int zkw_grand_product_chains(zkw_ctx* ctx, const uint64_t* lhs, const uint64_t* rhs, size_t n, int width,
                                        const uint64_t* challenges, int n_reps, uint64_t* lhs_z, uint64_t* rhs_z) {
    if (!ctx || !challenges || (n && (!lhs || !rhs || !lhs_z || !rhs_z)))
        return fail(ZKW_ERR_INVALID, "zkw_grand_product_chains: null argument");
    if ((width != 8 && width != 20) || (n_reps != 1 && n_reps != 2))
        return fail(ZKW_ERR_INVALID, "zkw_grand_product_chains: width must be 8 or 20, n_reps 1 or 2");
    HIP_TRY(hipSetDevice(ctx->device));
    if (n == 0) return ZKW_OK;
    const u64 *d_l = nullptr, *d_r = nullptr, *d_c = nullptr;
    u64 *d_lz = nullptr, *d_rz = nullptr;
    ZKW_TRY(ctx->in("gp_lhs", lhs, n * width, &d_l));
    ZKW_TRY(ctx->in("gp_rhs", rhs, n * width, &d_r));
    ZKW_TRY(ctx->in("gp_chal", challenges, (size_t)n_reps * (width + 1), &d_c));
    ZKW_TRY(ctx->out("gp_lz", lhs_z, n * n_reps, &d_lz));
    ZKW_TRY(ctx->out("gp_rz", rhs_z, n * n_reps, &d_rz));
    std::vector<GpSeg> segs(2);
    segs[0] = GpSeg{d_l, d_lz, d_c, n, 0, 0};
    segs[1] = GpSeg{d_r, d_rz, d_c, n, 0, 0};
    ZKW_TRY(dev_grand_products(ctx, segs, width, n_reps));
    ZKW_TRY(ctx->finish_out(lhs_z, d_lz, n * n_reps));
    ZKW_TRY(ctx->finish_out(rhs_z, d_rz, n * n_reps));
    ZKW_TRY(ctx->sync_if_host());
    if (ctx->ptr_mode == ZKW_PTR_HOST)
        for (int r = 0; r < n_reps; r++)
            if (lhs_z[(size_t)r * n + n - 1] != rhs_z[(size_t)r * n + n - 1])
                return fail(ZKW_ERR_CHECK_FAILED, "grand products differ in repetition %d (utils.rs:685-696)", r);
    return ZKW_OK;
}

extern "C" int zkw_encode_log_queries(zkw_ctx* ctx, const zkw_log_query* q, size_t n, const uint32_t* ext_ts,
                                      uint64_t* enc) {
    if (!ctx || (n && (!q || !enc))) return fail(ZKW_ERR_INVALID, "zkw_encode_log_queries: null argument");
    HIP_TRY(hipSetDevice(ctx->device));
    if (n == 0) return ZKW_OK;
    const zkw_log_query* d_q = nullptr;
    const u32* d_e = nullptr;
    u64* d_enc = nullptr;
    ZKW_TRY(ctx->in("lenc_q", q, n, &d_q));
    if (ext_ts) ZKW_TRY(ctx->in("lenc_ts", ext_ts, n, &d_e));
    ZKW_TRY(ctx->out("lenc_out", enc, n * 20, &d_enc));
    { Prof _p(ctx, "k_encode_log"); ZKW_LAUNCH(ctx, k_encode_log, blocks_for(n, 256), 256, d_q, n, d_e, d_enc); }
    ZKW_TRY(launch_check("k_encode_log"));
    ZKW_TRY(ctx->finish_out(enc, d_enc, n * 20));
    return ctx->sync_if_host();
}

extern "C" int zkw_encode_decommit_queries(zkw_ctx* ctx, const zkw_decommit_query* q, size_t n, uint64_t* enc) {
    if (!ctx || (n && (!q || !enc))) return fail(ZKW_ERR_INVALID, "zkw_encode_decommit_queries: null argument");
    HIP_TRY(hipSetDevice(ctx->device));
    if (n == 0) return ZKW_OK;
    const zkw_decommit_query* d_q = nullptr;
    u64* d_enc = nullptr;
    ZKW_TRY(ctx->in("denc_q", q, n, &d_q));
    ZKW_TRY(ctx->out("denc_out", enc, n * 8, &d_enc));
    { Prof _p(ctx, "k_encode_decommit"); ZKW_LAUNCH(ctx, k_encode_decommit, blocks_for(n, 256), 256, d_q, n, d_enc); }
    ZKW_TRY(launch_check("k_encode_decommit"));
    ZKW_TRY(ctx->finish_out(enc, d_enc, n * 8));
    return ctx->sync_if_host();
}

int dev_log_chains(zkw_ctx* ctx, const u64* d_enc, size_t total, std::vector<LogChainJob>& jobs) {
    const int key = ctx->chain_service && !ctx->batched() ? ctx->next_chain_key() : 0;
    if (total == 0 || jobs.empty()) { if (ctx->chain_service && !ctx->batched()) chain_service_of(ctx->device)->skip(key); return ZKW_OK; }
    u64* d_pre = nullptr;
    ZKW_TRY(ctx->scratch_t<u64>("log_pre", total * 4, &d_pre));
    { Prof _p(ctx, "k_log_prehash"); ZKW_LAUNCH(ctx, k_log_prehash, blocks_for(total, 128), 128, d_enc, total, d_pre); }
    ZKW_TRY(launch_check("k_log_prehash"));
    for (auto& j : jobs) j.pre = d_pre + (j.enc - d_enc) / 20 * 4;
    if (ctx->batched()) return zkw_batch_chains(ctx->batch, nullptr, 0, jobs.data(), jobs.size());
    if (ctx->chain_service) return chain_service_run(ctx, nullptr, &jobs, "k_chain_log", key);
    LogChainJob* d_jobs = nullptr;
    ZKW_TRY(ctx->upload("log_chain_jobs", jobs, &d_jobs));
    const int n_jobs = (int)jobs.size();
    { Prof _p(ctx, "k_chain_log"); hipLaunchKernelGGL(k_chain_log, dim3((n_jobs + 3) / 4), dim3(64), 0, ctx->stream, d_jobs, n_jobs); }
    return launch_check("k_chain_log");
}

extern "C" int zkw_queue_push_chain_log_batch(zkw_ctx* ctx, const uint64_t* enc, const uint64_t* offsets,
                                              size_t n_queues, const uint64_t* tails_in, uint64_t* old_tails,
                                              uint64_t* new_tails) {
    if (!ctx || !offsets) return fail(ZKW_ERR_INVALID, "zkw_queue_push_chain_log_batch: null argument");
    HIP_TRY(hipSetDevice(ctx->device));
    for (size_t k = 0; k < n_queues; k++)
        if (offsets[k + 1] < offsets[k]) return fail(ZKW_ERR_INVALID, "offsets must be non-decreasing");
    const size_t base = n_queues ? offsets[0] : 0, total = n_queues ? offsets[n_queues] - base : 0;
    if (total && (!enc || !new_tails)) return fail(ZKW_ERR_INVALID, "null enc/new_tails");
    const u64 *d_enc = nullptr, *d_tin = nullptr;
    u64 *d_old = nullptr, *d_new = nullptr;
    ZKW_TRY(ctx->in("lchain_enc", enc + base * 20, total * 20, &d_enc));
    if (tails_in) ZKW_TRY(ctx->in("lchain_tin", tails_in, n_queues * 4, &d_tin));
    if (old_tails) ZKW_TRY(ctx->out("lchain_old", old_tails + base * 4, total * 4, &d_old));
    ZKW_TRY(ctx->out("lchain_new", new_tails + base * 4, total * 4, &d_new));
    std::vector<LogChainJob> jobs(n_queues);
    for (size_t k = 0; k < n_queues; k++) {
        const size_t lo = offsets[k] - base;
        jobs[k] = LogChainJob{d_enc + lo * 20, nullptr, d_old ? d_old + lo * 4 : nullptr, d_new + lo * 4,
                              d_tin ? d_tin + 4 * k : nullptr, offsets[k + 1] - offsets[k]};
    }
    ZKW_TRY(dev_log_chains(ctx, d_enc, total, jobs));
    if (old_tails) ZKW_TRY(ctx->finish_out(old_tails + base * 4, d_old, total * 4));
    ZKW_TRY(ctx->finish_out(new_tails + base * 4, d_new, total * 4));
    return ctx->sync_if_host();
}

extern "C" int zkw_queue_push_chain_log(zkw_ctx* ctx, const uint64_t* enc, size_t n, const uint64_t tail_in[4],
                                        uint64_t* old_tails, uint64_t* new_tails) {
    uint64_t offsets[2] = {0, n};
    return zkw_queue_push_chain_log_batch(ctx, enc, offsets, 1, tail_in, old_tails, new_tails);
}

struct zkw_ram_witness {
    zkw_ctx* ctx = nullptr;
    std::vector<uint64_t> offsets;
    std::vector<uint64_t> inst_offsets;
    uint32_t capacity = 0;
    size_t total = 0, n_instances = 0;
    zkw_mem_query* sorted_q = nullptr;
    bool sorted_valid = false;
    u32* perm = nullptr;
    const zkw_mem_query* unsorted_q = nullptr;
    zkw_mem_query* owned_q = nullptr;
    u64 *unsorted_enc = nullptr, *sorted_enc = nullptr;
    bool enc_valid = false;
    u64 *unsorted_caps = nullptr, *sorted_caps = nullptr, *unsorted_marks = nullptr, *sorted_marks = nullptr;
    u64 *unsorted_tails = nullptr, *sorted_tails = nullptr;
    bool tails_valid = false;
    u64 *challenges = nullptr, *lhs_z = nullptr, *rhs_z = nullptr;
    bool z_valid = false;
    u64 *zbuf_l = nullptr, *zbuf_r = nullptr;
    u64* gp_ckpt = nullptr;
    u32* nd_prefix = nullptr;
    zkw_mem_query* sq_win = nullptr;
    size_t zcap = 0, sqcap = 0;
    zkw_ram_instance* instances = nullptr;
    u32* nondet_counts = nullptr;
    u64 *compact_forms = nullptr, *public_inputs = nullptr;

    void release() {
        void* ptrs[] = {sorted_q, perm, owned_q, unsorted_enc, sorted_enc, unsorted_caps, sorted_caps, unsorted_marks, sorted_marks,
                        unsorted_tails, sorted_tails, challenges,
                        lhs_z,    rhs_z,        instances,  nondet_counts, compact_forms, public_inputs, zbuf_l, zbuf_r, sq_win, gp_ckpt, nd_prefix};
        for (void* p : ptrs)
            if (p) dev_free(p);
        sorted_q = nullptr;
        sorted_valid = false;
        perm = nullptr;
        owned_q = nullptr;
        unsorted_q = nullptr;
        enc_valid = false;
        unsorted_enc = sorted_enc = unsorted_tails = sorted_tails = challenges = lhs_z = rhs_z = nullptr;
        unsorted_caps = sorted_caps = unsorted_marks = sorted_marks = nullptr;
        tails_valid = false;
        z_valid = false;
        zbuf_l = zbuf_r = nullptr;
        gp_ckpt = nullptr;
        nd_prefix = nullptr;
        sq_win = nullptr;
        zcap = sqcap = 0;
        instances = nullptr;
        nondet_counts = nullptr;
        compact_forms = public_inputs = nullptr;
    }
};

extern "C" void zkw_ram_witness_free(zkw_ram_witness* w);
static inline size_t ram_gp_groups(uint32_t capacity) { return ((size_t)capacity + 63) / 64; }
static inline size_t ram_nd_tiles(uint32_t capacity) { return ((size_t)capacity + 255) / 256; }
static int ram_alloc(zkw_ram_witness* w, size_t n_blocks) {
    const size_t t = w->total, ni = w->n_instances;
    HIP_TRY(dev_malloc((void**)&w->perm, (t + 1) * sizeof(u32)));
    HIP_TRY(dev_malloc((void**)&w->unsorted_caps, (t + 1) * 4 * sizeof(u64)));
    HIP_TRY(dev_malloc((void**)&w->sorted_caps, (t + 1) * 4 * sizeof(u64)));
    HIP_TRY(dev_malloc((void**)&w->unsorted_marks, (ni + 1) * 12 * sizeof(u64)));
    HIP_TRY(dev_malloc((void**)&w->sorted_marks, (ni + 1) * 12 * sizeof(u64)));
    HIP_TRY(dev_malloc((void**)&w->challenges, (n_blocks + 1) * 18 * sizeof(u64)));
    {
        size_t max_block = 0;
        for (size_t b = 0; b + 1 < w->offsets.size(); b++) max_block = std::max(max_block, (size_t)(w->offsets[b + 1] - w->offsets[b]));
        size_t window = (size_t)1 << 26, sq_window = (size_t)1 << 22;
        if (const char* e = getenv("ZKW_Z_WINDOW_ITEMS")) window = sq_window = (size_t)strtoull(e, nullptr, 10);
        w->zcap = std::max(max_block, std::min(t, window));
        w->sqcap = std::max(max_block, std::min(t, sq_window));
        HIP_TRY(dev_malloc((void**)&w->zbuf_l, (w->zcap + 1) * 2 * sizeof(u64)));
        HIP_TRY(dev_malloc((void**)&w->zbuf_r, (w->zcap + 1) * 2 * sizeof(u64)));
        HIP_TRY(dev_malloc((void**)&w->sq_win, (w->sqcap + 1) * sizeof(zkw_mem_query)));
    }
    HIP_TRY(dev_malloc((void**)&w->gp_ckpt, (ni * ram_gp_groups(w->capacity) + 1) * 4 * sizeof(u64)));
    HIP_TRY(dev_malloc((void**)&w->nd_prefix, (ni * ram_nd_tiles(w->capacity) + 1) * sizeof(u32)));
    HIP_TRY(dev_malloc((void**)&w->instances, (ni + 1) * sizeof(zkw_ram_instance)));
    HIP_TRY(dev_malloc((void**)&w->nondet_counts, (ni + 1) * sizeof(u32)));
    HIP_TRY(dev_malloc((void**)&w->compact_forms, (ni + 1) * COMPACT_FORM_LEN * sizeof(u64)));
    HIP_TRY(dev_malloc((void**)&w->public_inputs, (ni + 1) * 4 * sizeof(u64)));
    return ZKW_OK;
}

__device__ __forceinline__ u32 block_of_position(const u64* __restrict__ offsets, int n_blocks, size_t i) {
    int lo = 0, hi = n_blocks;
    while (hi - lo > 1) {
        int mid = (lo + hi) >> 1;
        if (offsets[mid] <= i) lo = mid; else hi = mid;
    }
    return (u32)lo;
}

static __device__ __forceinline__ void k_ram_key_ranges(const VB& vb, const zkw_mem_query* __restrict__ q, size_t n, u32* __restrict__ maxima) {
    u32 t = 0, p = 0, x = 0;
    for (size_t i = (size_t)vb.x * blockDim.x + threadIdx.x; i < n; i += (size_t)vb.nx * blockDim.x) {
        t = max(t, q[i].timestamp);
        p = max(p, q[i].page);
        x = max(x, q[i].index);
    }
    for (int o = 32; o > 0; o >>= 1) {
        t = max(t, (u32)__shfl_xor((int)t, o));
        p = max(p, (u32)__shfl_xor((int)p, o));
        x = max(x, (u32)__shfl_xor((int)x, o));
    }
    if ((threadIdx.x & 63) == 0) {
        atomicMax(maxima + 0, t);
        atomicMax(maxima + 1, p);
        atomicMax(maxima + 2, x);
    }
}

static __device__ __forceinline__ void k_ram_packed_keys(const VB& vb, const zkw_mem_query* __restrict__ q, size_t n, const u64* __restrict__ offsets,
                                  int n_blocks, unsigned bits_p, unsigned bits_i, unsigned bits_t,
                                  u64* __restrict__ key, u32* __restrict__ iota) {
    size_t i = (size_t)vb.x * blockDim.x + threadIdx.x;
    if (i >= n) return;
    u64 k = n_blocks > 1 ? block_of_position(offsets, n_blocks, i) : 0;
    k = (k << bits_p) | q[i].page;
    k = (k << bits_i) | q[i].index;
    k = (k << bits_t) | q[i].timestamp;
    key[i] = k;
    iota[i] = (u32)i;
}

static __device__ __forceinline__ void k_ram_packed_cells(const VB& vb, const u64* __restrict__ cell, const u32* __restrict__ perm, size_t n,
                                   const u64* __restrict__ offsets, int n_blocks, unsigned bits_p, unsigned bits_i,
                                   u64* __restrict__ key) {
    size_t i = (size_t)vb.x * blockDim.x + threadIdx.x;
    if (i >= n) return;
    const u32 src = perm[i];
    const u64 c = cell[src];
    u64 k = n_blocks > 1 ? block_of_position(offsets, n_blocks, src) : 0;
    k = (k << bits_p) | (c >> 32);
    k = (k << bits_i) | (c & 0xFFFFFFFFu);
    key[i] = k;
}

static __device__ __forceinline__ void k_block_ids(const VB& vb, const u64* __restrict__ offsets, int n_blocks, size_t n, u32* __restrict__ ids) {
    size_t i = (size_t)vb.x * blockDim.x + threadIdx.x;
    if (i < n) ids[i] = block_of_position(offsets, n_blocks, i);
}

static unsigned bits_in_use(u32 x) { return x ? 32u - (unsigned)__builtin_clz(x) : 0u; }

static int ram_sort(zkw_ctx* ctx, const zkw_mem_query* d_q, size_t total, const std::vector<uint64_t>& offsets,
                    void* work_a, void* work_b, u32** perm_out) {
    const size_t n_blocks = offsets.size() - 1;
    size_t tmp_bytes = radix_temp_bytes(total);
    u32* ts = static_cast<u32*>(work_a);
    u32 *k32 = ts + total, *v0 = k32 + total, *v1 = v0 + total;
    u64* cell = reinterpret_cast<u64*>(v1 + total);
    u64* k64a = cell + total;
    u64* k64b = static_cast<u64*>(work_b);
    void* tmp = nullptr;
    const size_t tmp_off = (total * 8 + 255) & ~(size_t)255;
    if (tmp_off + tmp_bytes <= total * 32) tmp = static_cast<char*>(work_b) + tmp_off;
    else ZKW_TRY(ctx->scratch("sort_tmp", tmp_bytes + 256, &tmp));
    const unsigned grid = blocks_for(total, 256);

    void* d_max_v = nullptr;
    ZKW_TRY(ctx->scratch("sort_max", 256, &d_max_v));
    u32* d_max = static_cast<u32*>(d_max_v);
    HIP_TRY(ctx->memset_async(d_max, 0, 16));
    { Prof _p(ctx, "k_ram_key_ranges");
      const unsigned g = grid < 4096 ? grid : 4096;
      ZKW_LAUNCH(ctx, k_ram_key_ranges, g, 256, d_q, total, d_max); }
    ZKW_TRY(launch_check("k_ram_key_ranges"));
    u32 maxima[4];
    ZKW_TRY(ctx->read_small(maxima, d_max, 16));
    const unsigned bits_t = bits_in_use(maxima[0]), bits_p = bits_in_use(maxima[1]), bits_i = bits_in_use(maxima[2]);
    unsigned bits_b = 0;
    while ((1ull << bits_b) < n_blocks) bits_b++;
    u64* d_off = nullptr;
    if (n_blocks > 1) ZKW_TRY(ctx->upload("sort_off", offsets, &d_off));

    if (bits_b + bits_p + bits_i + bits_t <= 64) {
        const unsigned bits = bits_b + bits_p + bits_i + bits_t;
        { Prof _p(ctx, "k_ram_packed_keys");
          ZKW_LAUNCH(ctx, k_ram_packed_keys, grid, 256, d_q, total, d_off, (int)n_blocks, bits_p, bits_i, bits_t, k64a, v0); }
        ZKW_TRY(launch_check("k_ram_packed_keys"));
        { Prof _p(ctx, "radix_sort"); ZKW_TRY(radix_sort_pairs<u64>(ctx, tmp, tmp_bytes, k64a, k64b, v0, v1, total, bits ? bits : 1)); }
        *perm_out = v1;
        return ZKW_OK;
    }

    { Prof _p(ctx, "k_ram_sort_keys"); ZKW_LAUNCH(ctx, k_ram_sort_keys, grid, 256, d_q, total, ts, cell, v0, (const u64*)nullptr, 0); }
    ZKW_TRY(launch_check("k_ram_sort_keys"));
    { Prof _p(ctx, "radix_sort"); ZKW_TRY(radix_sort_pairs<u32>(ctx, tmp, tmp_bytes, ts, k32, v0, v1, total, bits_t ? bits_t : 1)); }
    if (bits_b + bits_p + bits_i <= 64) {
        const unsigned bits = bits_b + bits_p + bits_i;
        { Prof _p(ctx, "k_ram_packed_cells");
          ZKW_LAUNCH(ctx, k_ram_packed_cells, grid, 256, cell, v1, total, d_off, (int)n_blocks, bits_p, bits_i, k64a); }
        ZKW_TRY(launch_check("k_ram_packed_cells"));
        { Prof _p(ctx, "radix_sort"); ZKW_TRY(radix_sort_pairs<u64>(ctx, tmp, tmp_bytes, k64a, k64b, v1, v0, total, bits ? bits : 1)); }
        *perm_out = v0;
        return ZKW_OK;
    }
    { Prof _p(ctx, "k_gather_u64_by_u32"); ZKW_LAUNCH(ctx, k_gather_u64_by_u32, grid, 256, cell, v1, total, k64a); }
    ZKW_TRY(launch_check("k_gather_u64_by_u32"));
    { Prof _p(ctx, "radix_sort"); ZKW_TRY(radix_sort_pairs<u64>(ctx, tmp, tmp_bytes, k64a, k64b, v1, v0, total, 64)); }
    { Prof _p(ctx, "k_block_ids"); ZKW_LAUNCH(ctx, k_block_ids, grid, 256, d_off, (int)n_blocks, total, ts); }
    ZKW_TRY(launch_check("k_block_ids"));
    { Prof _p(ctx, "k_gather_u32_by_u32"); ZKW_LAUNCH(ctx, k_gather_u32_by_u32, grid, 256, ts, v0, total, k32); }
    ZKW_TRY(launch_check("k_gather_u32_by_u32"));
    { Prof _p(ctx, "radix_sort"); ZKW_TRY(radix_sort_pairs<u32>(ctx, tmp, tmp_bytes, k32, ts, v0, v1, total, bits_b)); }
    *perm_out = v1;
    return ZKW_OK;
}

static int ram_gp_blocks(zkw_ctx* ctx, const zkw_ram_witness* w, size_t b0, size_t b1, u64* dst_l, u64* dst_r) {
    std::vector<GpSeg> segs;
    segs.reserve(2 * (b1 - b0));
    const size_t base = w->offsets[b0];
    for (size_t b = b0; b < b1; b++) {
        const size_t lo = w->offsets[b], n = w->offsets[b + 1] - lo;
        segs.push_back(GpSeg{nullptr, dst_l + 2 * (lo - base), w->challenges + 18 * b, n, 0, 0, w->unsorted_q + lo});
        segs.push_back(GpSeg{nullptr, dst_r + 2 * (lo - base), w->challenges + 18 * b, n, 0, 0, w->unsorted_q, w->perm + lo});
    }
    return dev_grand_products(ctx, segs, 8, 2);
}

static int ram_run(zkw_ctx* ctx, zkw_ram_witness* w, const zkw_mem_query* d_q, const uint32_t* n_nondet) {
    const size_t n_blocks = w->offsets.size() - 1, total = w->total;
    if (ctx->ptr_mode == ZKW_PTR_DEVICE) {
        w->unsorted_q = d_q;
    } else {
        if (!w->owned_q) HIP_TRY(dev_malloc((void**)&w->owned_q, (total + 1) * sizeof(zkw_mem_query)));
        HIP_TRY(ctx->copy_async(w->owned_q, d_q, total * sizeof(zkw_mem_query), hipMemcpyDeviceToDevice));
        w->unsorted_q = w->owned_q;
    }
    u32* perm = nullptr;
    ZKW_TRY(ram_sort(ctx, d_q, total, w->offsets, w->unsorted_caps, w->sorted_caps, &perm));
    w->tails_valid = false;
    w->enc_valid = false;
    w->sorted_valid = false;
    HIP_TRY(ctx->copy_async(w->perm, perm, total * sizeof(u32), hipMemcpyDeviceToDevice));
    std::vector<ChainJob> chains;
    chains.reserve(2 * n_blocks);
    for (size_t b = 0; b < n_blocks; b++) {
        const size_t lo = w->offsets[b], n = w->offsets[b + 1] - lo;
        const size_t io = w->inst_offsets[b];
        chains.push_back(ChainJob{nullptr, nullptr, nullptr, n, w->unsorted_caps + 4 * lo, w->unsorted_marks + 12 * io, w->capacity, w->unsorted_q + lo});
        chains.push_back(ChainJob{nullptr, nullptr, nullptr, n, w->sorted_caps + 4 * lo, w->sorted_marks + 12 * io, w->capacity, w->unsorted_q, w->perm + lo});
    }
    ZKW_TRY(dev_chains(ctx, chains));
    std::vector<FsJob> fs(n_blocks);
    for (size_t b = 0; b < n_blocks; b++) {
        const size_t lo = w->offsets[b], n = w->offsets[b + 1] - lo;
        const size_t last_inst = w->inst_offsets[b + 1] - 1;
        fs[b] = FsJob{w->unsorted_marks + 12 * last_inst, w->sorted_marks + 12 * last_inst, (u32)n, (u32)n,
                      w->challenges + 18 * b};
    }
    ZKW_TRY(dev_fs(ctx, fs, 12, 9));
    w->z_valid = false;
    for (size_t b0 = 0; b0 < n_blocks;) {
        size_t b1 = b0 + 1;
        while (b1 < n_blocks && w->offsets[b1 + 1] - w->offsets[b0] <= w->zcap) b1++;
        ZKW_TRY(ram_gp_blocks(ctx, w, b0, b1, w->zbuf_l, w->zbuf_r));
        const size_t base = w->offsets[b0];
        std::vector<RamBlock> blocks(b1 - b0);
        size_t max_inst = 0;
        for (size_t b = b0; b < b1; b++) {
            const size_t lo = w->offsets[b], n = w->offsets[b + 1] - lo;
            const size_t n_inst = w->inst_offsets[b + 1] - w->inst_offsets[b];
            if (n_inst > max_inst) max_inst = n_inst;
            blocks[b - b0] = RamBlock{w->unsorted_q,
                                      w->perm + lo,
                                      w->unsorted_marks + 12 * w->inst_offsets[b],
                                      w->sorted_marks + 12 * w->inst_offsets[b],
                                      w->zbuf_l + 2 * (lo - base),
                                      w->zbuf_r + 2 * (lo - base),
                                      w->instances + w->inst_offsets[b],
                                      w->nondet_counts + w->inst_offsets[b],
                                      w->gp_ckpt + 4 * ram_gp_groups(w->capacity) * w->inst_offsets[b],
                                      w->nd_prefix + ram_nd_tiles(w->capacity) * w->inst_offsets[b],
                                      n,
                                      w->capacity,
                                      n_nondet ? n_nondet[b] : 0u};
        }
        RamBlock* d_blocks = nullptr;
        ZKW_TRY(ctx->upload("ram_blocks", blocks, &d_blocks));
        const unsigned gx = (unsigned)(max_inst < 64 ? max_inst : 64), gy = (unsigned)(b1 - b0);
        { Prof _p(ctx, "k_ram_count_nondet"); ZKW_LAUNCH_2D(ctx, k_ram_count_nondet, gx, gy, 256, d_blocks); }
        ZKW_TRY(launch_check("k_ram_count_nondet"));
        { Prof _p(ctx, "k_ram_instances"); ZKW_LAUNCH_2D(ctx, k_ram_instances, blocks_for(max_inst, 64), gy, 64, d_blocks); }
        ZKW_TRY(launch_check("k_ram_instances"));
        { Prof _p(ctx, "k_ram_gp_ckpt"); ZKW_LAUNCH_2D(ctx, k_ram_gp_ckpt, blocks_for(max_inst * ram_gp_groups(w->capacity), 256), gy, 256, d_blocks); }
        ZKW_TRY(launch_check("k_ram_gp_ckpt"));
        b0 = b1;
    }
    const size_t ni = w->n_instances;
    { Prof _p(ctx, "k_ram_commitments"); ZKW_LAUNCH(ctx, k_ram_commitments, blocks_for(4 * ni, 64), 64, w->instances, ni, w->compact_forms); }
    ZKW_TRY(launch_check("k_ram_commitments"));
    { Prof _p(ctx, "k_commit_encodings"); ZKW_LAUNCH(ctx, k_commit_encodings, blocks_for(ni, 64), 64, w->compact_forms, ni, (u32)COMPACT_FORM_LEN, w->public_inputs); }
    return launch_check("k_commit_encodings");
}

extern "C" int zkw_ram_build_instances_batch(zkw_ctx* ctx, const zkw_mem_query* q, const uint64_t* block_offsets,
                                             size_t n_blocks, uint32_t capacity, const uint32_t* n_nondet,
                                             zkw_ram_witness** out) {
    if (!ctx || !q || !block_offsets || !out || n_blocks == 0 || capacity == 0)
        return fail(ZKW_ERR_INVALID, "zkw_ram_build_instances_batch: bad argument");
    HIP_TRY(hipSetDevice(ctx->device));
    const uint64_t base = block_offsets[0];
    std::vector<uint64_t> offs(n_blocks + 1), ioffs(n_blocks + 1, 0);
    for (size_t b = 0; b <= n_blocks; b++) offs[b] = block_offsets[b] - base;
    for (size_t b = 0; b < n_blocks; b++) {
        if (block_offsets[b + 1] <= block_offsets[b])
            return fail(ZKW_ERR_INVALID, "block %zu is empty: the VM must have made memory requests "
                                         "(W/ram_permutation.rs:43-46)", b);
        ioffs[b + 1] = ioffs[b] + (offs[b + 1] - offs[b] + capacity - 1) / capacity;
    }
    const size_t total = offs[n_blocks];
    if (total >= (1ull << 32)) return fail(ZKW_ERR_INVALID, "more than 2^32-1 queries in one batch");
    zkw_ram_witness* w = *out;
    if (w && (w->ctx != ctx || w->offsets != offs || w->capacity != capacity)) {
        zkw_ram_witness_free(w);
        w = nullptr;
        *out = nullptr;
    }
    if (!w) {
        w = new zkw_ram_witness();
        w->ctx = ctx;
        w->offsets = offs;
        w->inst_offsets = ioffs;
        w->capacity = capacity;
        w->total = total;
        w->n_instances = ioffs[n_blocks];
        int rc = ram_alloc(w, n_blocks);
        if (rc != ZKW_OK) {
            w->release();
            delete w;
            return rc;
        }
    }
    const zkw_mem_query* d_q = nullptr;
    int rc = ctx->in("ram_q", q + base, total, &d_q);
    if (rc == ZKW_OK) rc = ram_run(ctx, w, d_q, n_nondet);
    if (rc == ZKW_OK) rc = ctx->sync_if_host();
    if (rc != ZKW_OK) {
        if (!*out) {
            w->release();
            delete w;
        }
        return rc;
    }
    if (!*out) ctx_retain(ctx);
    *out = w;
    return ZKW_OK;
}

extern "C" int zkw_ram_build_instances(zkw_ctx* ctx, const zkw_mem_query* q, size_t n, uint32_t capacity,
                                       uint32_t num_non_deterministic_heap_queries, zkw_ram_witness** out) {
    uint64_t offsets[2] = {0, n};
    return zkw_ram_build_instances_batch(ctx, q, offsets, 1, capacity, &num_non_deterministic_heap_queries, out);
}

extern "C" size_t zkw_ram_witness_num_instances(const zkw_ram_witness* w) { return w ? w->n_instances : 0; }
extern "C" size_t zkw_ram_witness_num_items(const zkw_ram_witness* w) { return w ? w->total : 0; }

static int ram_sorted_queries(const zkw_ram_witness* cw) {
    zkw_ram_witness* w = const_cast<zkw_ram_witness*>(cw);
    if (w->sorted_valid) return ZKW_OK;
    zkw_ctx* ctx = w->ctx;
    HIP_TRY(hipSetDevice(ctx->device));
    const size_t t = w->total;
    if (!w->sorted_q && dev_malloc((void**)&w->sorted_q, (t + 1) * sizeof(zkw_mem_query)) != hipSuccess)
        return fail(ZKW_ERR_OOM, "no room for the sorted queries (%zu bytes): read ZKW_RAM_SORTED_QUERIES from a smaller batch", t * sizeof(zkw_mem_query));
    { Prof _p(ctx, "k_gather_encode"); ZKW_LAUNCH(ctx, k_gather_encode, blocks_for(t, 256), 256, w->unsorted_q, w->perm, t, w->sorted_q, (u64*)nullptr); }
    ZKW_TRY(launch_check("k_gather_encode"));
    w->sorted_valid = true;
    return ZKW_OK;
}

static int ram_full_chains(const zkw_ram_witness* cw) {
    zkw_ram_witness* w = const_cast<zkw_ram_witness*>(cw);
    if (w->z_valid) return ZKW_OK;
    zkw_ctx* ctx = w->ctx;
    HIP_TRY(hipSetDevice(ctx->device));
    const size_t t = w->total;
    if (!w->lhs_z) {
        if (dev_malloc((void**)&w->lhs_z, (t + 1) * 16) != hipSuccess || dev_malloc((void**)&w->rhs_z, (t + 1) * 16) != hipSuccess)
            return fail(ZKW_ERR_OOM, "no room for the grand-product chains (%zu bytes): read ZKW_RAM_*_Z from a smaller batch", 2 * t * 16);
    }
    ZKW_TRY(ram_gp_blocks(ctx, w, 0, w->offsets.size() - 1, w->lhs_z, w->rhs_z));
    w->z_valid = true;
    return ZKW_OK;
}

static int ram_encodings(const zkw_ram_witness* cw) {
    zkw_ram_witness* w = const_cast<zkw_ram_witness*>(cw);
    if (w->enc_valid) return ZKW_OK;
    zkw_ctx* ctx = w->ctx;
    HIP_TRY(hipSetDevice(ctx->device));
    const size_t t = w->total;
    if (!w->unsorted_enc) {
        if (dev_malloc((void**)&w->unsorted_enc, (t + 1) * 64) != hipSuccess || dev_malloc((void**)&w->sorted_enc, (t + 1) * 64) != hipSuccess)
            return fail(ZKW_ERR_OOM, "no room for the materialised encodings (%zu bytes): read ZKW_RAM_*_ENC from a smaller batch", 2 * t * 64);
    }
    ZKW_TRY(ram_sorted_queries(cw));
    ZKW_TRY(dev_encode(ctx, w->unsorted_q, t, w->unsorted_enc));
    ZKW_TRY(dev_encode(ctx, w->sorted_q, t, w->sorted_enc));
    w->enc_valid = true;
    return ZKW_OK;
}

static int ram_full_tails(const zkw_ram_witness* cw) {
    zkw_ram_witness* w = const_cast<zkw_ram_witness*>(cw);
    if (w->tails_valid) return ZKW_OK;
    ZKW_TRY(ram_encodings(cw));
    zkw_ctx* ctx = w->ctx;
    HIP_TRY(hipSetDevice(ctx->device));
    const size_t t = w->total;
    if (!w->unsorted_tails) {
        if (dev_malloc((void**)&w->unsorted_tails, (t + 1) * 96) != hipSuccess || dev_malloc((void**)&w->sorted_tails, (t + 1) * 96) != hipSuccess)
            return fail(ZKW_ERR_OOM, "no room for the expanded queue tails (%zu bytes): read ZKW_RAM_*_TAILS from a smaller batch", 2 * t * 96);
    }
    u64* d_off = nullptr;
    ZKW_TRY(ctx->upload("tails_off", w->offsets, &d_off));
    const int nq = (int)(w->offsets.size() - 1);
    { Prof _p(ctx, "k_tails_expand"); ZKW_LAUNCH(ctx, k_tails_expand, blocks_for(t, 64), 64, w->unsorted_enc, w->unsorted_caps, d_off, nq, t, w->unsorted_tails); }
    ZKW_TRY(launch_check("k_tails_expand"));
    { Prof _p(ctx, "k_tails_expand"); ZKW_LAUNCH(ctx, k_tails_expand, blocks_for(t, 64), 64, w->sorted_enc, w->sorted_caps, d_off, nq, t, w->sorted_tails); }
    ZKW_TRY(launch_check("k_tails_expand"));
    w->tails_valid = true;
    return ZKW_OK;
}

static const void* ram_array(const zkw_ram_witness* w, int what, size_t* bytes, bool materialize = true, int* rc = nullptr) {
    const size_t t = w->total, nb = w->offsets.size() - 1;
    int st = ZKW_OK;
    const void* p = nullptr;
#define RAM_LAZY(fn, field) do { if (materialize) { st = fn(w); if (st == ZKW_OK) p = w->field; } } while (0)
    switch (what) {
        case ZKW_RAM_SORTED_QUERIES: *bytes = t * sizeof(zkw_mem_query); RAM_LAZY(ram_sorted_queries, sorted_q); break;
        case ZKW_RAM_UNSORTED_ENC: *bytes = t * 64; RAM_LAZY(ram_encodings, unsorted_enc); break;
        case ZKW_RAM_SORTED_ENC: *bytes = t * 64; RAM_LAZY(ram_encodings, sorted_enc); break;
        case ZKW_RAM_UNSORTED_TAILS: *bytes = t * 96; RAM_LAZY(ram_full_tails, unsorted_tails); break;
        case ZKW_RAM_SORTED_TAILS: *bytes = t * 96; RAM_LAZY(ram_full_tails, sorted_tails); break;
        case ZKW_RAM_CHALLENGES: *bytes = nb * 18 * 8; p = w->challenges; break;
        case ZKW_RAM_LHS_Z: *bytes = t * 16; RAM_LAZY(ram_full_chains, lhs_z); break;
        case ZKW_RAM_RHS_Z: *bytes = t * 16; RAM_LAZY(ram_full_chains, rhs_z); break;
        case ZKW_RAM_INSTANCES: *bytes = w->n_instances * sizeof(zkw_ram_instance); p = w->instances; break;
        case ZKW_RAM_COMPACT_FORMS: *bytes = w->n_instances * COMPACT_FORM_LEN * 8; p = w->compact_forms; break;
        case ZKW_RAM_PUBLIC_INPUTS: *bytes = w->n_instances * 32; p = w->public_inputs; break;
        case ZKW_RAM_GP_CKPT: *bytes = w->n_instances * ram_gp_groups(w->capacity) * 32; p = w->gp_ckpt; break;
        case ZKW_RAM_ND_PREFIX: *bytes = w->n_instances * ram_nd_tiles(w->capacity) * sizeof(u32); p = w->nd_prefix; break;
        default: *bytes = 0; st = ZKW_ERR_INVALID; break;
    }
#undef RAM_LAZY
    if (rc) *rc = st;
    return p;
}

extern "C" size_t zkw_ram_witness_bytes(const zkw_ram_witness* w, int what) {
    size_t b = 0;
    if (w) (void)ram_array(w, what, &b, false);
    return b;
}

extern "C" const void* zkw_ram_witness_device_ptr(const zkw_ram_witness* w, int what) {
    size_t b = 0;
    return w ? ram_array(w, what, &b) : nullptr;
}

extern "C" int zkw_ram_witness_get(const zkw_ram_witness* w, int what, void* dst, size_t dst_bytes) {
    if (!w || !dst) return fail(ZKW_ERR_INVALID, "zkw_ram_witness_get: null argument");
    size_t bytes = 0;
    int st = ZKW_OK;
    const void* src = ram_array(w, what, &bytes, true, &st);
    if (st == ZKW_ERR_INVALID) return fail(ZKW_ERR_INVALID, "zkw_ram_witness_get: unknown array %d", what);
    if (st != ZKW_OK) return st;
    if (!src) return fail(ZKW_ERR_INVALID, "zkw_ram_witness_get: array %d is empty", what);
    if (dst_bytes < bytes) return fail(ZKW_ERR_INVALID, "zkw_ram_witness_get: need %zu bytes, got %zu", bytes, dst_bytes);
    zkw_ctx* ctx = w->ctx;
    HIP_TRY(hipSetDevice(ctx->device));
    HIP_TRY(ctx->copy_async(dst, src, bytes, ctx->ptr_mode == ZKW_PTR_DEVICE ? hipMemcpyDeviceToDevice : hipMemcpyDeviceToHost));
    return ctx->sync_if_host();
}

extern "C" void zkw_ram_witness_free(zkw_ram_witness* w) {
    if (!w) return;
    (void)hipSetDevice(w->ctx->device);
    (void)hipStreamSynchronize(w->ctx->stream);
    w->release();
    zkw_ctx* owner = w->ctx;
    delete w;
    ctx_release(owner);
}


extern "C" int zkw_trace_create_with_columns(zkw_ctx* ctx, size_t n_rows, size_t n_cols, size_t n_slots, zkw_trace** out) {
    if (!ctx || !out || n_rows < 256 || n_slots == 0 || n_cols == 0 || n_cols > 4096)
        return fail(ZKW_ERR_INVALID, "zkw_trace_create: bad argument");
    HIP_TRY(hipSetDevice(ctx->device));
    zkw_trace* t = new zkw_trace();
    t->ctx = ctx;
    t->n_rows = n_rows;
    t->n_cols = n_cols;
    t->n_slots = n_slots;
    t->slot_tag.reset(new std::atomic<uint64_t>[n_slots]);
    for (size_t k = 0; k < n_slots; k++) t->slot_tag[k].store(0, std::memory_order_relaxed);
    hipError_t e = dev_malloc((void**)&t->data, t->slot_elems() * n_slots * sizeof(u64));
    if (e != hipSuccess) {
        delete t;
        return fail(ZKW_ERR_OOM, "zkw_trace_create: hipMalloc of %zu bytes failed: %s",
                    n_cols * n_rows * n_slots * 8, hipGetErrorString(e));
    }
    ctx_retain(ctx);
    *out = t;
    return ZKW_OK;
}

extern "C" int zkw_trace_create(zkw_ctx* ctx, size_t n_rows, size_t n_slots, zkw_trace** out) {
    return zkw_trace_create_with_columns(ctx, n_rows, RC_COLS, n_slots, out);
}

extern "C" void zkw_trace_free(zkw_trace* t) {
    if (!t) return;
    (void)hipSetDevice(t->ctx->device);
    (void)hipStreamSynchronize(t->ctx->stream);
    if (t->data) dev_free(t->data);
    zkw_ctx* owner = t->ctx;
    delete t;
    ctx_release(owner);
}

extern "C" size_t zkw_trace_num_rows(const zkw_trace* t) { return t ? t->n_rows : 0; }
extern "C" size_t zkw_trace_num_cols(const zkw_trace* t) { return t ? t->n_cols : 0; }
extern "C" size_t zkw_trace_num_slots(const zkw_trace* t) { return t ? t->n_slots : 0; }
extern "C" const uint64_t* zkw_trace_device_ptr(const zkw_trace* t, size_t slot) {
    if (!t || slot >= t->n_slots) return nullptr;
    return t->slot_for_write(slot, 0);
}

extern "C" int zkw_trace_get(const zkw_trace* t, size_t slot, uint32_t first_col, uint32_t n_cols, uint64_t* dst) {
    if (!t || !dst || slot >= t->n_slots || (size_t)first_col + n_cols > t->n_cols) return fail(ZKW_ERR_INVALID, "zkw_trace_get: bad argument");
    zkw_ctx* ctx = t->ctx;
    HIP_TRY(hipSetDevice(ctx->device));
    const u64* src = t->data + slot * t->slot_elems() + (size_t)first_col * t->n_rows;
    HIP_TRY(ctx->copy_async(dst, src, (size_t)n_cols * t->n_rows * sizeof(u64), ctx->ptr_mode == ZKW_PTR_DEVICE ? hipMemcpyDeviceToDevice : hipMemcpyDeviceToHost));
    return ctx->sync_if_host();
}

extern "C" int zkw_ram_synthesize(zkw_ctx* ctx, const zkw_ram_witness* w, size_t first_instance, size_t n_instances,
                                  zkw_trace* t, size_t first_slot) {
    if (!ctx || !w || !t || w->ctx != ctx || t->ctx->device != ctx->device) return fail(ZKW_ERR_INVALID, "zkw_ram_synthesize: bad argument");
    if (first_instance + n_instances > w->n_instances) return fail(ZKW_ERR_INVALID, "instance range out of bounds");
    if (n_instances > t->n_slots) return fail(ZKW_ERR_INVALID, "more instances (%zu) than trace slots (%zu)", n_instances, t->n_slots);
    const u32 capacity = w->capacity;
    const size_t n_rows = t->n_rows;
    if (RC_MIN_ROWS(capacity) > n_rows)
        return fail(ZKW_ERR_INVALID, "capacity %u needs %llu rows, trace has %zu", capacity,
                    (unsigned long long)RC_MIN_ROWS(capacity), n_rows);
    if (n_rows & 1) return fail(ZKW_ERR_INVALID, "trace length must be even (it is a power of two in every circuit)");
    if (n_instances == 0) return ZKW_OK;
    HIP_TRY(hipSetDevice(ctx->device));
    const size_t n_blocks = w->offsets.size() - 1;
    size_t b_first = 0;
    while (b_first + 1 < n_blocks && w->inst_offsets[b_first + 1] <= first_instance) b_first++;
    size_t b_end = b_first + 1;
    while (b_end < n_blocks && w->inst_offsets[b_end] < first_instance + n_instances) b_end++;
    const size_t win = w->sqcap;
    if (w->offsets[b_end] - w->offsets[b_first] > win) {
        size_t b_mid = b_first + 1;
        while (b_mid + 1 < b_end && w->offsets[b_mid + 1] - w->offsets[b_first] <= win) b_mid++;
        const size_t n_head = w->inst_offsets[b_mid] - first_instance;
        ZKW_TRY(zkw_ram_synthesize(ctx, w, first_instance, n_head, t, first_slot));
        return zkw_ram_synthesize(ctx, w, first_instance + n_head, n_instances - n_head, t, first_slot + n_head);
    }
    const size_t z_base = w->offsets[b_first];
    {
        const size_t cnt = w->offsets[b_end] - z_base;
        Prof _p(ctx, "k_gather_encode");
        ZKW_LAUNCH(ctx, k_gather_encode, blocks_for(cnt, 256), 256, w->unsorted_q, w->perm + z_base, cnt, w->sq_win, (u64*)nullptr);
    }
    ZKW_TRY(launch_check("k_gather_encode"));
    const u32 rstride = (u32)RC_REGION_STRIDE(capacity);
    const u32 n_tiles = (rstride + 255) / 256;
    u32* d_hist = nullptr;
    {
        const DevBuf& hb = ctx->pool["synth_hist"];
        const void* had = hb.p;
        ZKW_TRY(ctx->scratch_t<u32>("synth_hist", n_instances * 256, &d_hist));
        if (hb.p != had || ctx->synth_hist_dirty) HIP_TRY(ctx->memset_async(hb.p, 0, hb.cap));
        ctx->synth_hist_dirty = true;
    }
    SlotClaims claims(t);
    const bool inline_jobs = n_instances <= (size_t)RC_INLINE_JOBS && !ctx->batched();
    SynthJobsInline tab;
    std::vector<SynthJob> jobs(inline_jobs ? 0 : n_instances);
    bool all_clean = true;
    size_t b = b_first;
    for (size_t k = 0; k < n_instances; k++) {
        const size_t idx = first_instance + k;
        while (b + 1 < n_blocks && w->inst_offsets[b + 1] <= idx) b++;
        const size_t lo = w->offsets[b];
        SynthJob& j = inline_jobs ? tab.j[k] : jobs[k];
        j.inst = w->instances + idx;
        j.sorted_q = w->sq_win + (lo - z_base);
        j.unsorted_q = w->unsorted_q + lo;
        j.unsorted_caps = w->unsorted_caps + 4 * lo;
        j.sorted_caps = w->sorted_caps + 4 * lo;
        j.u_mark = w->unsorted_marks + 12 * idx;
        j.s_mark = w->sorted_marks + 12 * idx;
        j.challenges = w->challenges + 18 * b;
        j.gp_ckpt = w->gp_ckpt + 4 * ram_gp_groups(capacity) * idx;
        {
            const uint64_t tag = ((uint64_t)ZKW_CIRCUIT_RAM_PERMUTATION << 56) ^ ((uint64_t)capacity << 24) ^ (uint64_t)n_rows ^ 0x5A00000000000000ull;
            const size_t slot = (first_slot + k) % t->n_slots;
            bool clean = false;
            j.trace = claims.claim(slot, tag, &clean);
            j.tail_clean = clean;
            all_clean = all_clean && clean;
        }
        j.hist = d_hist + 256 * k;
        j.nd_tiles = w->nd_prefix + (size_t)n_tiles * idx;
        j.public_input = w->public_inputs + 4 * idx;
        j.first_inst = w->instances + w->inst_offsets[b];
    }
    SynthJobsRef ref{nullptr};
    if (!inline_jobs) {
        SynthJob* d_jobs = nullptr;
        ZKW_TRY(ctx->upload("synth_jobs", jobs, &d_jobs));
        ref.p = d_jobs;
    } else {
        for (size_t k = n_instances; k < (size_t)RC_INLINE_JOBS; k++) tab.j[k] = tab.j[0];
    }
#define SYNTH_LAUNCH(kernel, name, grid, bs, ...)                                                                                  \
    do {                                                                                                                           \
        if (inline_jobs) {                                                                                                         \
            LaunchSig<decltype(&kernel<SynthJobsInline>)>::template single<&kernel<SynthJobsInline>, bs>(ctx->stream, grid, 0, tab, __VA_ARGS__); \
            ZKW_TRY(launch_check(name));                                                                                           \
        } else {                                                                                                                   \
            ZKW_LAUNCH_D(ctx, (kernel<SynthJobsRef>), name, grid, bs, 0, ref, __VA_ARGS__);                                        \
        }                                                                                                                          \
    } while (0)
    const unsigned nj = (unsigned)n_instances;
    const dim3 g64x2((rstride + 63) / 64, nj, 2), g256(n_tiles, nj);
    { Prof _p(ctx, "k_ram_fill_C"); SYNTH_LAUNCH(k_ram_fill_C, "k_ram_fill_C", g256, 256, capacity, n_rows); }
    { Prof _p(ctx, "k_ram_fill_poseidon", 2); SYNTH_LAUNCH(k_ram_fill_poseidon, "k_ram_fill_poseidon", g64x2, 64, capacity, n_rows); }
    { Prof _p(ctx, "k_ram_fill_D"); const unsigned d_tiles = (unsigned)((rstride + RC_D_TILES * 256 - 1) / (RC_D_TILES * 256));
      SYNTH_LAUNCH(k_ram_fill_D, "k_ram_fill_D", dim3(nj * (d_tiles + 1)), 256, nj, d_tiles, capacity, n_rows); }
    ctx->synth_hist_dirty = false;
    if (!all_clean) { Prof _p(ctx, "k_ram_fill_tail"); SYNTH_LAUNCH(k_ram_fill_tail, "k_ram_fill_tail", dim3(nj * ((RC_G + RC_L + 1) * TAIL_CHUNKS)), 256, capacity, n_rows); }
#undef SYNTH_LAUNCH
    return claims.commit_if(ctx->sync_if_host());
}


extern "C" int zkw_ram_check_satisfied(zkw_ctx* ctx, const zkw_trace* t, size_t slot, uint32_t capacity,
                                       uint64_t* n_violations, uint64_t* first_bad) {
    if (!ctx || !t || t->ctx->device != ctx->device || slot >= t->n_slots || !n_violations)
        return fail(ZKW_ERR_INVALID, "zkw_ram_check_satisfied: bad argument");
    if (RC_MIN_ROWS(capacity) > t->n_rows) return fail(ZKW_ERR_INVALID, "capacity does not fit the trace");
    return check_satisfied<SpecRam>(ctx, t, slot, capacity, n_violations, first_bad);
}

extern "C" int zkw_decommit_sorter_check_satisfied(zkw_ctx* ctx, const zkw_trace* t, size_t slot, uint32_t capacity,
                                                   uint64_t* n_violations, uint64_t* first_bad) {
    if (!ctx || !t || t->ctx->device != ctx->device || slot >= t->n_slots || !n_violations)
        return fail(ZKW_ERR_INVALID, "zkw_decommit_sorter_check_satisfied: bad argument");
    if (DS_MIN_ROWS(capacity) > t->n_rows) return fail(ZKW_ERR_INVALID, "capacity does not fit the trace");
    return check_satisfied<SpecDecommitSorter>(ctx, t, slot, capacity, n_violations, first_bad);
}

extern "C" int zkw_closed_form_public_inputs(zkw_ctx* ctx, uint8_t circuit_type, const void* instances, size_t n, uint64_t* compact,
                                             uint64_t* public_inputs) {
    if (!ctx || !compact || !public_inputs || (n && !instances)) return fail(ZKW_ERR_INVALID, "zkw_closed_form_public_inputs: null argument");
    if (n == 0) return ZKW_OK;
    HIP_TRY(hipSetDevice(ctx->device));
    switch (circuit_type) {
        case 3: return closed_form_from_records<CfDecommitter>(ctx, instances, n, compact, public_inputs);
        case 5: return closed_form_from_records<CfPrecompile<ZKW_PRECOMPILE_KECCAK256>>(ctx, instances, n, compact, public_inputs);
        case 6: return closed_form_from_records<CfPrecompile<ZKW_PRECOMPILE_SHA256>>(ctx, instances, n, compact, public_inputs);
        case 7: return closed_form_from_records<CfPrecompile<ZKW_PRECOMPILE_ECRECOVER>>(ctx, instances, n, compact, public_inputs);
        case 10: return closed_form_from_records<CfStorageApplication>(ctx, instances, n, compact, public_inputs);
        case 13: return closed_form_from_records<CfLinearHasher>(ctx, instances, n, compact, public_inputs);
        default: break;
    }
    return fail(ZKW_ERR_INVALID, "zkw_closed_form_public_inputs: circuit type %u keeps its compact forms in its witness (2, 4, 8, 9, 11, 12) "
                                 "or is not a base-layer circuit with a closed form here", (unsigned)circuit_type);
}

extern "C" int zkw_commit_encodings(zkw_ctx* ctx, const uint64_t* enc, size_t n_items, uint32_t item_len, uint64_t* out) {
    if (!ctx || !out || (n_items && item_len && !enc)) return fail(ZKW_ERR_INVALID, "zkw_commit_encodings: null argument");
    if (n_items == 0) return ZKW_OK;
    HIP_TRY(hipSetDevice(ctx->device));
    const u64* d_enc = nullptr;
    u64* d_out = nullptr;
    ZKW_TRY(ctx->in("ce_enc", enc, n_items * item_len + 1, &d_enc));
    ZKW_TRY(ctx->out("ce_out", out, n_items * 4, &d_out));
    { Prof _p(ctx, "k_commit_encodings"); ZKW_LAUNCH(ctx, k_commit_encodings, blocks_for(n_items, 64), 64, d_enc, n_items, item_len, d_out); }
    ZKW_TRY(launch_check("k_commit_encodings"));
    ZKW_TRY(ctx->finish_out(out, d_out, n_items * 4));
    return ctx->sync_if_host();
}

extern "C" int zkw_encode_recursion_requests(zkw_ctx* ctx, uint64_t circuit_type, const uint64_t* public_inputs, size_t n,
                                             uint64_t* enc) {
    if (!ctx || !enc || !public_inputs) return fail(ZKW_ERR_INVALID, "zkw_encode_recursion_requests: null argument");
    if (n == 0) return ZKW_OK;
    HIP_TRY(hipSetDevice(ctx->device));
    const u64* d_pi = nullptr;
    u64* d_enc = nullptr;
    ZKW_TRY(ctx->in("rr_pi", public_inputs, n * 4, &d_pi));
    ZKW_TRY(ctx->out("rr_enc", enc, n * 8, &d_enc));
    { Prof _p(ctx, "k_encode_recursion"); ZKW_LAUNCH(ctx, k_encode_recursion, blocks_for(n, 64), 64, circuit_type, d_pi, n, d_enc); }
    ZKW_TRY(launch_check("k_encode_recursion"));
    ZKW_TRY(ctx->finish_out(enc, d_enc, n * 8));
    return ctx->sync_if_host();
}

extern "C" int zkw_encode_callstack_entries(zkw_ctx* ctx, const zkw_callstack_entry* entries, size_t n, uint64_t* enc) {
    if (!ctx || !enc || !entries) return fail(ZKW_ERR_INVALID, "zkw_encode_callstack_entries: null argument");
    if (n == 0) return ZKW_OK;
    HIP_TRY(hipSetDevice(ctx->device));
    const zkw_callstack_entry* d_e = nullptr;
    u64* d_enc = nullptr;
    ZKW_TRY(ctx->in("cs_e", entries, n, &d_e));
    ZKW_TRY(ctx->out("cs_enc", enc, n * 32, &d_enc));
    { Prof _p(ctx, "k_encode_callstack"); hipLaunchKernelGGL(k_encode_callstack, dim3(blocks_for(n, 64)), dim3(64), 0, ctx->stream, d_e, n, d_enc); }
    ZKW_TRY(launch_check("k_encode_callstack"));
    ZKW_TRY(ctx->finish_out(enc, d_enc, n * 32));
    return ctx->sync_if_host();
}

extern "C" int zkw_callstack_simulate(zkw_ctx* ctx, const uint8_t* is_push, size_t n_ops, const zkw_callstack_entry* pushed,
                                      size_t n_pushed, uint64_t* previous_state, uint64_t* new_state, uint32_t* depth,
                                      uint64_t* round_states, uint32_t* entry_index) {
    if (!ctx || !is_push || !previous_state || !new_state || !depth || !round_states || !entry_index || (n_pushed && !pushed))
        return fail(ZKW_ERR_INVALID, "zkw_callstack_simulate: null argument");
    if (n_ops == 0) return ZKW_OK;
    if (n_ops >= (1ull << 31)) return fail(ZKW_ERR_INVALID, "too many stack operations");
    HIP_TRY(hipSetDevice(ctx->device));
    const uint8_t* d_ops = nullptr;
    const zkw_callstack_entry* d_e = nullptr;
    ZKW_TRY(ctx->in("st_ops", is_push, n_ops, &d_ops));
    if (n_pushed) ZKW_TRY(ctx->in("st_e", pushed, n_pushed, &d_e));
    u32 *d_depth = nullptr, *d_rank = nullptr, *d_meta = nullptr, *d_pd = nullptr, *d_pid = nullptr, *d_sd = nullptr, *d_sid = nullptr,
        *d_parent = nullptr, *d_node = nullptr;
    u64* d_rounds = nullptr;
    void* tmp = nullptr;
    const size_t tmp_bytes = radix_temp_bytes(n_ops);
    ZKW_TRY(ctx->scratch_t<u32>("st_depth", n_ops, &d_depth));
    ZKW_TRY(ctx->scratch_t<u32>("st_rank", n_ops, &d_rank));
    ZKW_TRY(ctx->scratch_t<u32>("st_meta", 4, &d_meta));
    ZKW_TRY(ctx->scratch_t<u32>("st_pd", n_ops, &d_pd));
    ZKW_TRY(ctx->scratch_t<u32>("st_pid", n_ops, &d_pid));
    ZKW_TRY(ctx->scratch_t<u32>("st_sd", n_ops, &d_sd));
    ZKW_TRY(ctx->scratch_t<u32>("st_sid", n_ops, &d_sid));
    ZKW_TRY(ctx->scratch_t<u32>("st_parent", n_ops, &d_parent));
    ZKW_TRY(ctx->scratch_t<u32>("st_node", n_ops, &d_node));
    ZKW_TRY(ctx->scratch_t<u64>("st_rounds", n_ops * 48, &d_rounds));
    ZKW_TRY(ctx->scratch("st_tmp", tmp_bytes + 256, &tmp));
    u64 *d_prefix = nullptr, *d_totals = nullptr;
    ZKW_TRY(ctx->scratch_t<u64>("st_prefix", 2 * (n_ops + 1), &d_prefix));
    ZKW_TRY(ctx->scratch_t<u64>("st_totals", 2, &d_totals));
    HIP_TRY(ctx->memset_async(d_meta, 0, 4 * sizeof(u32)));
    ZKW_TRY((sum_prefix<2>(ctx, "k_stack_prefix", StackDelta{d_ops}, n_ops, d_prefix, d_totals)));
    { Prof _p(ctx, "k_stack_depth"); hipLaunchKernelGGL(k_stack_depth, dim3(blocks_for(n_ops, 256)), dim3(256), 0, ctx->stream, d_ops, n_ops, d_prefix, d_depth, d_rank, d_meta); }
    ZKW_TRY(launch_check("k_stack_depth"));
    u32 meta[3];
    ZKW_TRY(ctx->read_small(meta, d_meta, sizeof meta));
    if (meta[2]) return fail(ZKW_ERR_INVALID, "pop from the empty callstack (circuit_encodings/src/lib.rs:619)");
    const u32 n_push = meta[0], max_depth = meta[1];
    if (n_push > n_pushed) return fail(ZKW_ERR_INVALID, "%u pushes but only %zu entries", n_push, n_pushed);
    const unsigned grid = blocks_for(n_ops, 256);
    if (n_push) {
        { Prof _p(ctx, "k_stack_push_keys"); hipLaunchKernelGGL(k_stack_push_keys, dim3(grid), dim3(256), 0, ctx->stream, d_ops, n_ops, d_depth, d_rank, d_pd, d_pid); }
        ZKW_TRY(launch_check("k_stack_push_keys"));
        unsigned bits = 1;
        while ((1ull << bits) <= max_depth) bits++;
        { Prof _p(ctx, "radix_sort"); ZKW_TRY(radix_sort_pairs<u32>(ctx, tmp, tmp_bytes, d_pd, d_sd, d_pid, d_sid, n_push, bits)); }
    }
    { Prof _p(ctx, "k_stack_links"); hipLaunchKernelGGL(k_stack_links, dim3(grid), dim3(256), 0, ctx->stream, d_ops, n_ops, d_depth, d_rank, d_sd, d_sid, d_meta, d_parent, d_node); }
    ZKW_TRY(launch_check("k_stack_links"));
    for (u32 d = 1; d <= max_depth; d++) {
        Prof _p(ctx, "k_stack_level");
        hipLaunchKernelGGL(k_stack_level, dim3(blocks_for(n_push, 64)), dim3(64), 0, ctx->stream, d_e, d_pd, d_parent, d_meta, d, d_rounds);
    }
    ZKW_TRY(launch_check("k_stack_level"));
    u64 *d_prev = nullptr, *d_new = nullptr, *d_rs = nullptr;
    u32 *d_dep = nullptr, *d_idx = nullptr;
    ZKW_TRY(ctx->out("st_o_prev", previous_state, n_ops * 12, &d_prev));
    ZKW_TRY(ctx->out("st_o_new", new_state, n_ops * 12, &d_new));
    ZKW_TRY(ctx->out("st_o_rs", round_states, n_ops * 48, &d_rs));
    ZKW_TRY(ctx->out("st_o_dep", depth, n_ops, &d_dep));
    ZKW_TRY(ctx->out("st_o_idx", entry_index, n_ops, &d_idx));
    { Prof _p(ctx, "k_stack_emit"); hipLaunchKernelGGL(k_stack_emit, dim3(grid), dim3(256), 0, ctx->stream, d_ops, n_ops, d_depth, d_parent, d_node, d_rounds, d_meta, d_prev, d_new, d_dep, d_rs, d_idx); }
    ZKW_TRY(launch_check("k_stack_emit"));
    ZKW_TRY(ctx->finish_out(previous_state, d_prev, n_ops * 12));
    ZKW_TRY(ctx->finish_out(new_state, d_new, n_ops * 12));
    ZKW_TRY(ctx->finish_out(round_states, d_rs, n_ops * 48));
    ZKW_TRY(ctx->finish_out(depth, d_dep, n_ops));
    ZKW_TRY(ctx->finish_out(entry_index, d_idx, n_ops));
    return ctx->sync_if_host();
}

extern "C" int zkw_vm_slice_instances(zkw_ctx* ctx, const zkw_vm_tracer_streams* in, zkw_vm_instance* instances,
                                      uint32_t* memory_read_index, uint32_t* memory_write_index, uint64_t* n_reads, uint64_t* n_writes) {
    if (!ctx || !in || !instances || !in->snapshot_cycles || in->n_snapshots < 2 || ((memory_read_index == nullptr) != (memory_write_index == nullptr)))
        return fail(ZKW_ERR_INVALID, "zkw_vm_slice_instances: bad argument");
    for (int k = 0; k < ZKW_VM_NUM_STREAMS; k++)
        if (in->stream_len[k] && !in->stream_cycles[k]) return fail(ZKW_ERR_INVALID, "zkw_vm_slice_instances: stream %d has no cycle stamps", k);
    const size_t n_mem = in->stream_len[ZKW_VMS_MEMORY];
    if (n_mem >= (1ull << 32)) return fail(ZKW_ERR_INVALID, "too many memory queries");
    if ((n_mem && (!in->vm_memory_queries || !in->memory_queue_tails)) || (in->n_decommit_states && (!in->decommit_state_cycles || !in->decommit_queue_tails)) ||
        (in->n_callstack_sponges && (!in->callstack_sponge_cycles || !in->callstack_sponge_states)) ||
        (in->n_storage_log_states && (!in->storage_log_state_cycles || !in->storage_log_states)))
        return fail(ZKW_ERR_INVALID, "zkw_vm_slice_instances: a stream's payload is missing");
    HIP_TRY(hipSetDevice(ctx->device));
    const size_t n_inst = in->n_snapshots - 1;
    VmSliceJob job;
    job.s = *in;
    ZKW_TRY(ctx->in("vm_snap", in->snapshot_cycles, in->n_snapshots, &job.s.snapshot_cycles));
    static const char* names[ZKW_VM_NUM_STREAMS] = {"vm_c0", "vm_c1", "vm_c2", "vm_c3", "vm_c4", "vm_c5", "vm_c6", "vm_c7"};
    for (int k = 0; k < ZKW_VM_NUM_STREAMS; k++) ZKW_TRY(ctx->in(names[k], in->stream_cycles[k], in->stream_len[k], &job.s.stream_cycles[k]));
    ZKW_TRY(ctx->in("vm_memq", in->vm_memory_queries, n_mem, &job.s.vm_memory_queries));
    ZKW_TRY(ctx->in("vm_memt", in->memory_queue_tails, n_mem * 12, &job.s.memory_queue_tails));
    ZKW_TRY(ctx->in("vm_decc", in->decommit_state_cycles, in->n_decommit_states, &job.s.decommit_state_cycles));
    ZKW_TRY(ctx->in("vm_dect", in->decommit_queue_tails, in->n_decommit_states * 12, &job.s.decommit_queue_tails));
    ZKW_TRY(ctx->in("vm_csc", in->callstack_sponge_cycles, in->n_callstack_sponges, &job.s.callstack_sponge_cycles));
    ZKW_TRY(ctx->in("vm_css", in->callstack_sponge_states, in->n_callstack_sponges * 12, &job.s.callstack_sponge_states));
    ZKW_TRY(ctx->in("vm_slc", in->storage_log_state_cycles, in->n_storage_log_states, &job.s.storage_log_state_cycles));
    ZKW_TRY(ctx->in("vm_sls", in->storage_log_states, in->n_storage_log_states, &job.s.storage_log_states));
    u32 *d_tiles = nullptr, *d_prefix = nullptr, *d_ri = nullptr, *d_wi = nullptr;
    u64* d_total = nullptr;
    const u32 n_tiles = (u32)((n_mem + VM_TILE) / VM_TILE);
    ZKW_TRY(ctx->scratch_t<u32>("vm_tiles", n_tiles, &d_tiles));
    ZKW_TRY(ctx->scratch_t<u32>("vm_prefix", n_mem + 1, &d_prefix));
    ZKW_TRY(ctx->scratch_t<u64>("vm_total", 1, &d_total));
    if (memory_read_index) {
        ZKW_TRY(ctx->out("vm_ri", memory_read_index, n_mem, &d_ri));
        ZKW_TRY(ctx->out("vm_wi", memory_write_index, n_mem, &d_wi));
    }
    { Prof _p(ctx, "k_vm_rw_tile_counts"); ZKW_LAUNCH(ctx, k_vm_rw_tile_counts, n_tiles, 256, job.s.vm_memory_queries, (u64)n_mem, d_tiles); }
    ZKW_TRY(launch_check("k_vm_rw_tile_counts"));
    { Prof _p(ctx, "k_vm_rw_scan_tiles"); ZKW_LAUNCH(ctx, k_vm_rw_scan_tiles, 1, 1024, d_tiles, n_tiles, d_total); }
    ZKW_TRY(launch_check("k_vm_rw_scan_tiles"));
    { Prof _p(ctx, "k_vm_rw_scatter"); ZKW_LAUNCH(ctx, k_vm_rw_scatter, n_tiles, 256, job.s.vm_memory_queries, (u64)n_mem, d_tiles, d_prefix, d_ri, d_wi); }
    ZKW_TRY(launch_check("k_vm_rw_scatter"));
    job.read_prefix = d_prefix;
    ZKW_TRY(ctx->out("vm_inst", instances, n_inst, &job.out));
    { Prof _p(ctx, "k_vm_slice"); ZKW_LAUNCH(ctx, k_vm_slice, blocks_for(n_inst, 64), 64, job); }
    ZKW_TRY(launch_check("k_vm_slice"));
    ZKW_TRY(ctx->finish_out(instances, job.out, n_inst));
    if (memory_read_index) {
        ZKW_TRY(ctx->finish_out(memory_read_index, d_ri, n_mem));
        ZKW_TRY(ctx->finish_out(memory_write_index, d_wi, n_mem));
    }
    if (n_reads || n_writes) {
        u64 total = 0;
        ZKW_TRY(ctx->read_small(&total, d_total, 8));
        if (n_reads) *n_reads = total;
        if (n_writes) *n_writes = n_mem - total;
    }
    return ctx->sync_if_host();
}
```

Measured before the change: 3496.

## Use segmented radix sort and fuse RAM grand-product with nondet counting

Adds a segmented radix sort that builds per-segment tiles from a segment table, so block IDs no longer go into the sort keys and the extra block-id sort pass is dropped. The RAM grand-product computation changes from a z-buffer pass plus a separate checkpoint kernel to one per-tile kernel. That kernel computes the challenge-weighted query encodings, reduces the products per 64-row group and counts nondeterministic queries in the same pass, and a single-block scan kernel then does the prefix products and prefix counts. The goal is fewer sort passes and less memory traffic. The cost is a serial per-block scan kernel and a binary search over the segment table in every sort tile.

```diff
diff --git a/era_zkevm_test_harness_amd/csrc/radix_sort.cuh b/era_zkevm_test_harness_amd/csrc/radix_sort.cuh
--- a/era_zkevm_test_harness_amd/csrc/radix_sort.cuh
+++ b/era_zkevm_test_harness_amd/csrc/radix_sort.cuh
@@ -8,20 +8,51 @@
 template <class K>
 static __device__ __forceinline__ unsigned rs_digit(K key, unsigned shift, unsigned mask) { return (unsigned)(key >> shift) & mask; }
 
-template <class K>
-static __device__ __forceinline__ void k_rs_hist(const VB& vb, const K* __restrict__ keys, size_t n, unsigned shift, unsigned mask, u32* __restrict__ hist, u32 n_tiles) {
+struct RsSeg {
+    u32 off, tile0;
+};
+
+static __device__ __forceinline__ void rs_seg_tile(const RsSeg* __restrict__ segs, u32 n_segs, u32 x, size_t& base, size_t& end, size_t& e0, u32& stride) {
+    u32 lo = 0, hi = n_segs;
+    while (hi - lo > 1) {
+        const u32 mid = (lo + hi) >> 1;
+        if (segs[mid].tile0 <= x) lo = mid; else hi = mid;
+    }
+    const RsSeg s = segs[lo], next = segs[lo + 1];
+    const u32 t = x - s.tile0;
+    stride = next.tile0 - s.tile0;
+    base = (size_t)s.off + (size_t)t * RS_TILE;
+    end = next.off;
+    e0 = (size_t)256 * s.tile0 + t;
+}
+
+template <class K>
+static __device__ __forceinline__ void rs_hist_tile(const K* __restrict__ keys, size_t base, size_t end, unsigned shift, unsigned mask, u32* __restrict__ h, size_t stride) {
     __shared__ u32 cnt[256];
     const int t = threadIdx.x;
     cnt[t] = 0;
     __syncthreads();
-    const size_t base = (size_t)vb.x * RS_TILE;
 #pragma unroll 4
     for (int r = 0; r < RS_TILE / 256; r++) {
         const size_t i = base + (size_t)r * 256 + t;
-        if (i < n) atomicAdd(&cnt[rs_digit(keys[i], shift, mask)], 1u);
-    }
-    __syncthreads();
-    hist[(size_t)t * n_tiles + vb.x] = cnt[t];
+        if (i < end) atomicAdd(&cnt[rs_digit(keys[i], shift, mask)], 1u);
+    }
+    __syncthreads();
+    h[(size_t)t * stride] = cnt[t];
+}
+
+template <class K>
+static __device__ __forceinline__ void k_rs_hist(const VB& vb, const K* __restrict__ keys, size_t n, unsigned shift, unsigned mask, u32* __restrict__ hist, u32 n_tiles) {
+    rs_hist_tile<K>(keys, (size_t)vb.x * RS_TILE, n, shift, mask, hist + vb.x, n_tiles);
+}
+
+template <class K>
+static __device__ __forceinline__ void k_rs_hist_seg(const VB& vb, const K* __restrict__ keys, const RsSeg* __restrict__ segs, u32 n_segs, unsigned shift, unsigned mask,
+                                                     u32* __restrict__ hist) {
+    size_t base, end, e0;
+    u32 stride;
+    rs_seg_tile(segs, n_segs, vb.x, base, end, e0, stride);
+    rs_hist_tile<K>(keys, base, end, shift, mask, hist + e0, stride);
 }
 
 static __device__ __forceinline__ void k_rs_scan_a(const VB& vb, u32* __restrict__ hist, size_t n_entries, u32* __restrict__ chunk_tot) {
@@ -80,8 +111,8 @@
 }
 
 template <class K>
-static __device__ __forceinline__ void k_rs_scatter(const VB& vb, const K* __restrict__ kin, const u32* __restrict__ vin, size_t n, unsigned shift, unsigned mask,
-                                    const u32* __restrict__ hist, const u32* __restrict__ chunk_off, u32 n_tiles, K* __restrict__ kout, u32* __restrict__ vout) {
+static __device__ __forceinline__ void rs_scatter_tile(const K* __restrict__ kin, const u32* __restrict__ vin, size_t tile0, size_t n, unsigned shift, unsigned mask,
+                                    const u32* __restrict__ hist, const u32* __restrict__ chunk_off, size_t e0, size_t stride, K* __restrict__ kout, u32* __restrict__ vout) {
     __shared__ K s_key[RS_TILE];
     __shared__ u32 s_val[RS_TILE];
     __shared__ u32 wcnt[RS_WAVES][256];
@@ -92,7 +123,7 @@
 #pragma unroll
     for (int w = 0; w < RS_WAVES; w++) wcnt[w][t] = 0;
     __syncthreads();
-    const size_t tile0 = (size_t)vb.x * RS_TILE, base = tile0 + (size_t)wave * (RS_ROUNDS * 64) + lane;
+    const size_t base = tile0 + (size_t)wave * (RS_ROUNDS * 64) + lane;
     K key[RS_ROUNDS];
     u32 val[RS_ROUNDS];
     unsigned long long same[RS_ROUNDS];
@@ -133,7 +164,7 @@
         u32 first = incl - total;
         for (int w = 0; w < wave; w++) first += s_wsum[w];
         s_first[t] = first;
-        const size_t e = (size_t)t * n_tiles + vb.x;
+        const size_t e = e0 + (size_t)t * stride;
         s_gbase[t] = hist[e] + chunk_off[e / RS_CHUNK] - first;
         u32 at = first;
 #pragma unroll
@@ -162,6 +193,22 @@
         kout[at] = k;
         vout[at] = s_val[p];
     }
+}
+
+template <class K>
+static __device__ __forceinline__ void k_rs_scatter(const VB& vb, const K* __restrict__ kin, const u32* __restrict__ vin, size_t n, unsigned shift, unsigned mask,
+                                    const u32* __restrict__ hist, const u32* __restrict__ chunk_off, u32 n_tiles, K* __restrict__ kout, u32* __restrict__ vout) {
+    rs_scatter_tile<K>(kin, vin, (size_t)vb.x * RS_TILE, n, shift, mask, hist, chunk_off, vb.x, n_tiles, kout, vout);
+}
+
+template <class K>
+static __device__ __forceinline__ void k_rs_scatter_seg(const VB& vb, const K* __restrict__ kin, const u32* __restrict__ vin, const RsSeg* __restrict__ segs, u32 n_segs,
+                                    unsigned shift, unsigned mask, const u32* __restrict__ hist, const u32* __restrict__ chunk_off, K* __restrict__ kout,
+                                    u32* __restrict__ vout) {
+    size_t base, end, e0;
+    u32 stride;
+    rs_seg_tile(segs, n_segs, vb.x, base, end, e0, stride);
+    rs_scatter_tile<K>(kin, vin, base, end, shift, mask, hist, chunk_off, e0, stride, kout, vout);
 }
 
 static inline size_t rs_tiles(size_t n) { return (n + RS_TILE - 1) / RS_TILE; }
@@ -202,4 +249,69 @@
     return ZKW_OK;
 }
 
-}
+
+static inline u32 rs_seg_table(const uint64_t* offsets, size_t n_segs, std::vector<RsSeg>& table) {
+    table.resize(n_segs + 1);
+    u32 tiles = 0;
+    for (size_t s = 0; s < n_segs; s++) {
+        table[s] = RsSeg{(u32)offsets[s], tiles};
+        tiles += (u32)rs_tiles(offsets[s + 1] - offsets[s]);
+    }
+    table[n_segs] = RsSeg{(u32)offsets[n_segs], tiles};
+    return tiles;
+}
+static inline size_t radix_temp_bytes(size_t n, size_t n_segs) {
+    const size_t entries = 256 * (n / RS_TILE + n_segs), chunks = (entries + RS_CHUNK - 1) / RS_CHUNK;
+    return ((n * 8 + 255) & ~(size_t)255) + ((n * 4 + 255) & ~(size_t)255) + entries * 4 + chunks * 4 + 1024;
+}
+
+template <class K>
+static int radix_sort_pairs_segmented(zkw_ctx* ctx, void* tmp, size_t tmp_bytes, const K* kin, K* kout, const u32* vin, u32* vout, size_t n, const RsSeg* d_segs,
+                                      u32 n_segs, u32 n_tiles, unsigned end_bit) {
+    if (n == 0) return ZKW_OK;
+    if (n >= (1ull << 32)) return fail(ZKW_ERR_INVALID, "radix_sort_pairs_segmented: more than 2^32 - 1 pairs");
+    if (n_segs == 0 || n_tiles > n / RS_TILE + n_segs) return fail(ZKW_ERR_INVALID, "radix_sort_pairs_segmented: the segment table does not belong to these pairs");
+    if (tmp_bytes < radix_temp_bytes(n, n_segs)) return fail(ZKW_ERR_INVALID, "radix_sort_pairs_segmented: temporary storage too small");
+    if (end_bit == 0) end_bit = 1;
+    const unsigned passes = (end_bit + 7) / 8;
+    const size_t entries = (size_t)256 * n_tiles;
+    const u32 n_chunks = (u32)((entries + RS_CHUNK - 1) / RS_CHUNK);
+    char* p = static_cast<char*>(tmp);
+    K* tk = reinterpret_cast<K*>(p);
+    u32* tv = reinterpret_cast<u32*>(p + ((n * 8 + 255) & ~(size_t)255));
+    u32* hist = reinterpret_cast<u32*>(p + ((n * 8 + 255) & ~(size_t)255) + ((n * 4 + 255) & ~(size_t)255));
+    u32* chunk = hist + entries;
+    const K* src_k = kin;
+    const u32* src_v = vin;
+    for (unsigned pass = 0; pass < passes; pass++) {
+        const bool to_out = ((passes - pass) & 1) == 1;
+        K* dst_k = to_out ? kout : tk;
+        u32* dst_v = to_out ? vout : tv;
+        const unsigned shift = 8 * pass, bits = std::min(8u, end_bit - shift), mask = (1u << bits) - 1;
+        ZKW_LAUNCH_T(ctx, (k_rs_hist_seg<K>), "k_rs_hist_seg", n_tiles, 256, src_k, d_segs, n_segs, shift, mask, hist);
+        ZKW_LAUNCH(ctx, k_rs_scan_a, n_chunks, 1024, hist, entries, chunk);
+        ZKW_LAUNCH(ctx, k_rs_scan_b, 1, 1024, chunk, n_chunks);
+        ZKW_LAUNCH_T(ctx, (k_rs_scatter_seg<K>), "k_rs_scatter_seg", n_tiles, 256, src_k, src_v, d_segs, n_segs, shift, mask, (const u32*)hist, (const u32*)chunk, dst_k, dst_v);
+        src_k = dst_k;
+        src_v = dst_v;
+    }
+    return ZKW_OK;
+}
+
+template <class K>
+static int radix_sort_pairs_segmented(zkw_ctx* ctx, void* tmp, size_t tmp_bytes, const K* kin, K* kout, const u32* vin, u32* vout, const uint64_t* offsets, size_t n_segs,
+                                      unsigned end_bit) {
+    if (n_segs == 0 || offsets[0] != 0) return fail(ZKW_ERR_INVALID, "radix_sort_pairs_segmented: bad segment offsets");
+    for (size_t s = 0; s < n_segs; s++)
+        if (offsets[s + 1] < offsets[s]) return fail(ZKW_ERR_INVALID, "radix_sort_pairs_segmented: bad segment offsets");
+    const size_t n = offsets[n_segs];
+    if (n == 0) return ZKW_OK;
+    if (n >= (1ull << 32)) return fail(ZKW_ERR_INVALID, "radix_sort_pairs_segmented: more than 2^32 - 1 pairs");
+    std::vector<RsSeg> table;
+    const u32 n_tiles = rs_seg_table(offsets, n_segs, table);
+    RsSeg* d_segs = nullptr;
+    ZKW_TRY(ctx->upload("rs_segs", table, &d_segs));
+    return radix_sort_pairs_segmented<K>(ctx, tmp, tmp_bytes, kin, kout, vin, vout, n, d_segs, (u32)n_segs, n_tiles, end_bit);
+}
+
+}
diff --git a/era_zkevm_test_harness_amd/csrc/ram_kernels.cuh b/era_zkevm_test_harness_amd/csrc/ram_kernels.cuh
--- a/era_zkevm_test_harness_amd/csrc/ram_kernels.cuh
+++ b/era_zkevm_test_harness_amd/csrc/ram_kernels.cuh
@@ -455,13 +455,14 @@
 struct RamBlock {
     const zkw_mem_query* sorted_q;
     const u32* sorted_perm;
+    const zkw_mem_query* unsorted_q;
+    const u64* chal;
     const u64* u_marks;
     const u64* s_marks;
-    const u64* lhs_z;
-    const u64* rhs_z;
     zkw_ram_instance* instances;
     u32* nondet_prefix;
     u64* gp_ckpt;
+    u64* gp_total;
     u32* nd_prefix;
     u64 n;
     u32 capacity;
@@ -472,35 +473,138 @@
     for (int k = 0; k < 12; k++) dst[k] = src[k];
 }
 
-static __device__ __forceinline__ void k_ram_count_nondet(const VB& vb, const RamBlock* __restrict__ blocks) {
+static __device__ __forceinline__ void k_ram_gp_groups(const VB& vb, const RamBlock* __restrict__ blocks) {
     const RamBlock b = blocks[vb.y];
     const u64 n_inst = (b.n + b.capacity - 1) / b.capacity;
+    const u32 n_tiles = (b.capacity + 255) / 256, groups = (b.capacity + 63) / 64;
+    const u64 inst = vb.x / n_tiles;
+    const u32 t = vb.x % n_tiles;
+    if (inst >= n_inst) return;
+    __shared__ u32 sh[4];
+    const int lane = threadIdx.x & 63, wave = threadIdx.x >> 6;
+    const u64 lo = inst * b.capacity, hi = lo + b.capacity < b.n ? lo + b.capacity : b.n;
+    const u64 i = lo + 256 * (u64)t + threadIdx.x;
+    const bool live = i < hi;
+    zkw_mem_query qs;
+    memset(&qs, 0, sizeof qs);
+    u64 eu[8], es[8];
+#pragma unroll
+    for (int k = 0; k < 8; k++) eu[k] = 0;
+    if (live) {
+        const RawQuery ru = load_raw_query(b.unsorted_q + i), rs = load_raw_query(b.sorted_q + b.sorted_perm[i]);
+        encode_raw_query(ru, eu);
+        uint4* d = reinterpret_cast<uint4*>(&qs);
+        d[0] = rs.a; d[1] = rs.b; d[2] = rs.c;
+    }
+    encode_mem_query(qs, es);
+    const bool f = live && qs.rw_flag && qs.timestamp == 0 && qs.page == ZKW_BOOTLOADER_HEAP_PAGE, fc = f && !qs.value_is_pointer;
+    u64 p[4];
+#pragma unroll
+    for (int r = 0; r < 2; r++) {
+        const u64* ch = b.chal + 9 * r;
+        u64 lc = ch[8], rc = ch[8];
+#pragma unroll
+        for (int k = 0; k < 8; k++) {
+            lc = gl::add(lc, gl::mul(eu[k], ch[k]));
+            rc = gl::add(rc, gl::mul(es[k], ch[k]));
+            __builtin_amdgcn_sched_barrier(0);
+        }
+        p[r] = live ? lc : 1;
+        p[2 + r] = live ? rc : 1;
+    }
+#pragma unroll
+    for (int d = 32; d > 0; d >>= 1) {
+#pragma unroll
+        for (int k = 0; k < 4; k += 2) {
+            const u64 o0 = __shfl_xor(p[k], d, 64), o1 = __shfl_xor(p[k + 1], d, 64);
+            p[k] = gl::mul(p[k], o0);
+            p[k + 1] = gl::mul(p[k + 1], o1);
+            __builtin_amdgcn_sched_barrier(0);
+        }
+    }
+    const u32 g = 4 * t + wave;
+    if (lane == 0 && g < groups) {
+        u64* out = b.gp_ckpt + 4 * (inst * groups + g);
+#pragma unroll
+        for (int k = 0; k < 4; k++) out[k] = gl::canon(p[k]);
+    }
+    const u32 c = (u32)__popcll(__ballot(f)) | (u32)__popcll(__ballot(fc)) << 16;
+    if (lane == 0) sh[wave] = c;
+    __syncthreads();
+    if (threadIdx.x == 0) b.nd_prefix[inst * n_tiles + t] = sh[0] + sh[1] + sh[2] + sh[3];
+}
+
+static __device__ __forceinline__ void k_ram_gp_scan(const VB& vb, const RamBlock* __restrict__ blocks) {
+    const RamBlock b = blocks[vb.y];
+    const u64 n_inst = (b.n + b.capacity - 1) / b.capacity, groups = (b.capacity + 63) / 64, total = n_inst * groups;
     const u32 n_tiles = (b.capacity + 255) / 256;
-    __shared__ u32 sh[2][2][4];
-    for (u64 inst = vb.x; inst < n_inst; inst += vb.nx) {
-        const u64 lo = inst * b.capacity, hi = lo + b.capacity < b.n ? lo + b.capacity : b.n;
-        u32 cnt = 0, before = 0;
-        for (u32 t = 0; t < n_tiles; t++) {
-            const u64 i = lo + 256 * (u64)t + threadIdx.x;
-            bool f = false, fc = false;
-            if (i < hi) {
-                const zkw_mem_query* q = b.sorted_q + b.sorted_perm[i];
-                f = q->rw_flag && q->timestamp == 0 && q->page == ZKW_BOOTLOADER_HEAP_PAGE;
-                fc = f && !q->value_is_pointer;
+    __shared__ u64 sh_w[4][4];
+    const int lane = threadIdx.x & 63, wave = threadIdx.x >> 6;
+    u64 carry[4];
+#pragma unroll
+    for (int k = 0; k < 4; k++) carry[k] = 1;
+    for (u64 base = 0; base < total; base += 256) {
+        const u64 j = base + threadIdx.x;
+        const bool ok = j < total;
+        u64* at = b.gp_ckpt + 4 * j;
+        u64 s[4];
+#pragma unroll
+        for (int k = 0; k < 4; k++) s[k] = ok ? at[k] : 1;
+#pragma unroll
+        for (int d = 1; d < 64; d <<= 1) {
+#pragma unroll
+            for (int k = 0; k < 4; k += 2) {
+                const u64 o0 = __shfl_up(s[k], d, 64), o1 = __shfl_up(s[k + 1], d, 64);
+                if (lane >= d) { s[k] = gl::mul(s[k], o0); s[k + 1] = gl::mul(s[k + 1], o1); }
+                __builtin_amdgcn_sched_barrier(0);
             }
-            const u32 c = __popcll(__ballot(f)), cc = __popcll(__ballot(fc));
-            if ((threadIdx.x & 63) == 0) { sh[t & 1][0][threadIdx.x >> 6] = c; sh[t & 1][1][threadIdx.x >> 6] = cc; }
-            __syncthreads();
-            if (threadIdx.x == 0) {
-                const u32* s0 = sh[t & 1][0];
-                const u32* s1 = sh[t & 1][1];
-                b.nd_prefix[inst * n_tiles + t] = before;
-                cnt += s0[0] + s0[1] + s0[2] + s0[3];
-                before += s1[0] + s1[1] + s1[2] + s1[3];
+        }
+        if (lane == 63) {
+#pragma unroll
+            for (int k = 0; k < 4; k++) sh_w[wave][k] = s[k];
+        }
+        __syncthreads();
+#pragma unroll
+        for (int k = 0; k < 4; k += 2) {
+            const u64 e0 = __shfl_up(s[k], 1, 64), e1 = __shfl_up(s[k + 1], 1, 64);
+            u64 pre0 = carry[k], pre1 = carry[k + 1], tot0 = carry[k], tot1 = carry[k + 1];
+#pragma unroll
+            for (int w = 0; w < 4; w++) {
+                tot0 = gl::mul(tot0, sh_w[w][k]);
+                tot1 = gl::mul(tot1, sh_w[w][k + 1]);
+                if (w + 1 == wave) { pre0 = tot0; pre1 = tot1; }
+                __builtin_amdgcn_sched_barrier(0);
             }
-        }
-        if (threadIdx.x == 0) b.nondet_prefix[inst] = cnt;
+            carry[k] = tot0;
+            carry[k + 1] = tot1;
+            const u64 x0 = lane == 0 ? pre0 : gl::mul(pre0, e0), x1 = lane == 0 ? pre1 : gl::mul(pre1, e1);
+            if (ok) { at[k] = gl::canon(x0); at[k + 1] = gl::canon(x1); }
+            __builtin_amdgcn_sched_barrier(0);
+        }
         __syncthreads();
+    }
+    if (threadIdx.x == 0) {
+#pragma unroll
+        for (int k = 0; k < 4; k++) b.gp_total[k] = gl::canon(carry[k]);
+    }
+    for (u64 inst = wave; inst < n_inst; inst += 4) {
+        u32* tiles = b.nd_prefix + inst * n_tiles;
+        u32 fsm = 0, before = 0;
+        for (u32 t0 = 0; t0 < n_tiles; t0 += 64) {
+            const u32 t = t0 + lane;
+            const u32 v = t < n_tiles ? tiles[t] : 0;
+            u32 incl = v;
+#pragma unroll
+            for (int d = 1; d < 64; d <<= 1) {
+                const u32 y = __shfl_up(incl, d, 64);
+                if (lane >= d) incl += y;
+            }
+            if (t < n_tiles) tiles[t] = before + ((incl - v) >> 16);
+            const u32 sum = __shfl(incl, 63, 64);
+            fsm += sum & 0xFFFFu;
+            before += sum >> 16;
+        }
+        if (lane == 0) b.nondet_prefix[inst] = fsm;
     }
 }
 
@@ -527,9 +631,10 @@
     u32 nondet_before = 0;
     for (u64 k = 0; k < idx; k++) nondet_before += b.nondet_prefix[k];
 
-    auto fill = [&](zkw_ram_fsm& f, u64 end , u32 nondet) {
+    const u64 groups = (b.capacity + 63) / 64;
+    auto fill = [&](zkw_ram_fsm& f, u64 end , u32 nondet, const u64* acc) {
         const u64 l = end - 1;
-        for (int r = 0; r < 2; r++) { f.lhs_accumulator[r] = b.lhs_z[r * n + l]; f.rhs_accumulator[r] = b.rhs_z[r * n + l]; }
+        for (int r = 0; r < 2; r++) { f.lhs_accumulator[r] = acc[r]; f.rhs_accumulator[r] = acc[2 + r]; }
         copy12(f.current_unsorted_queue_state.head, b.u_marks + 12 * (l / b.capacity));
         copy12(f.current_unsorted_queue_state.tail, u_final);
         f.current_unsorted_queue_state.length = (u32)(n - end);
@@ -546,31 +651,15 @@
     if (idx == 0) {
         for (int r = 0; r < 2; r++) { w.hidden_fsm_input.lhs_accumulator[r] = 1; w.hidden_fsm_input.rhs_accumulator[r] = 1; }
     } else {
-        fill(w.hidden_fsm_input, lo, nondet_before);
-    }
-    fill(w.hidden_fsm_output, hi, nondet_before + b.nondet_prefix[idx]);
+        fill(w.hidden_fsm_input, lo, nondet_before, b.gp_ckpt + 4 * groups * idx);
+    }
+    fill(w.hidden_fsm_output, hi, nondet_before + b.nondet_prefix[idx], idx + 1 < n_inst ? b.gp_ckpt + 4 * groups * (idx + 1) : b.gp_total);
     if ((hi - lo) % b.capacity != 0) {
         zkw_ram_fsm& f = w.hidden_fsm_output;
         for (int k = 0; k < 3; k++) f.previous_sorting_key[k] = 0;
         for (int k = 0; k < 2; k++) f.previous_full_key[k] = 0;
         for (int k = 0; k < 8; k++) f.previous_value[k] = 0;
         f.previous_is_ptr = 0;
-    }
-}
-
-static __device__ __forceinline__ void k_ram_gp_ckpt(const VB& vb, const RamBlock* __restrict__ blocks) {
-    const RamBlock b = blocks[vb.y];
-    const u64 n_inst = (b.n + b.capacity - 1) / b.capacity, groups = (b.capacity + 63) / 64;
-    const u64 j = (u64)vb.x * blockDim.x + threadIdx.x;
-    if (j >= n_inst * groups) return;
-    const u64 idx = j / groups, g = j % groups;
-    const zkw_ram_instance& in = b.instances[idx];
-    const u64 first = in.first_item, m = in.num_items;
-    u64* out = b.gp_ckpt + 4 * j;
-    for (int r = 0; r < 2; r++) {
-        const u64 at = (u64)r * b.n + first + (64 * g - 1 < m ? 64 * g - 1 : m - 1);
-        out[r] = g == 0 ? in.hidden_fsm_input.lhs_accumulator[r] : b.lhs_z[at];
-        out[2 + r] = g == 0 ? in.hidden_fsm_input.rhs_accumulator[r] : b.rhs_z[at];
     }
 }
 
diff --git a/era_zkevm_test_harness_amd/csrc/zkw_api.hip b/era_zkevm_test_harness_amd/csrc/zkw_api.hip
--- a/era_zkevm_test_harness_amd/csrc/zkw_api.hip
+++ b/era_zkevm_test_harness_amd/csrc/zkw_api.hip
@@ -957,11 +957,10 @@
     bool tails_valid = false;
     u64 *challenges = nullptr, *lhs_z = nullptr, *rhs_z = nullptr;
     bool z_valid = false;
-    u64 *zbuf_l = nullptr, *zbuf_r = nullptr;
-    u64* gp_ckpt = nullptr;
+    u64 *gp_ckpt = nullptr, *gp_total = nullptr;
     u32* nd_prefix = nullptr;
     zkw_mem_query* sq_win = nullptr;
-    size_t zcap = 0, sqcap = 0;
+    size_t sqcap = 0;
     zkw_ram_instance* instances = nullptr;
     u32* nondet_counts = nullptr;
     u64 *compact_forms = nullptr, *public_inputs = nullptr;
@@ -969,7 +968,7 @@
     void release() {
         void* ptrs[] = {sorted_q, perm, owned_q, unsorted_enc, sorted_enc, unsorted_caps, sorted_caps, unsorted_marks, sorted_marks,
                         unsorted_tails, sorted_tails, challenges,
-                        lhs_z,    rhs_z,        instances,  nondet_counts, compact_forms, public_inputs, zbuf_l, zbuf_r, sq_win, gp_ckpt, nd_prefix};
+                        lhs_z,    rhs_z,        instances,  nondet_counts, compact_forms, public_inputs, sq_win, gp_ckpt, gp_total, nd_prefix};
         for (void* p : ptrs)
             if (p) dev_free(p);
         sorted_q = nullptr;
@@ -982,11 +981,10 @@
         unsorted_caps = sorted_caps = unsorted_marks = sorted_marks = nullptr;
         tails_valid = false;
         z_valid = false;
-        zbuf_l = zbuf_r = nullptr;
-        gp_ckpt = nullptr;
+        gp_ckpt = gp_total = nullptr;
         nd_prefix = nullptr;
         sq_win = nullptr;
-        zcap = sqcap = 0;
+        sqcap = 0;
         instances = nullptr;
         nondet_counts = nullptr;
         compact_forms = public_inputs = nullptr;
@@ -1007,30 +1005,19 @@
     {
         size_t max_block = 0;
         for (size_t b = 0; b + 1 < w->offsets.size(); b++) max_block = std::max(max_block, (size_t)(w->offsets[b + 1] - w->offsets[b]));
-        size_t window = (size_t)1 << 26, sq_window = (size_t)1 << 22;
-        if (const char* e = getenv("ZKW_Z_WINDOW_ITEMS")) window = sq_window = (size_t)strtoull(e, nullptr, 10);
-        w->zcap = std::max(max_block, std::min(t, window));
+        size_t sq_window = (size_t)1 << 22;
+        if (const char* e = getenv("ZKW_Z_WINDOW_ITEMS")) sq_window = (size_t)strtoull(e, nullptr, 10);
         w->sqcap = std::max(max_block, std::min(t, sq_window));
-        HIP_TRY(dev_malloc((void**)&w->zbuf_l, (w->zcap + 1) * 2 * sizeof(u64)));
-        HIP_TRY(dev_malloc((void**)&w->zbuf_r, (w->zcap + 1) * 2 * sizeof(u64)));
         HIP_TRY(dev_malloc((void**)&w->sq_win, (w->sqcap + 1) * sizeof(zkw_mem_query)));
     }
     HIP_TRY(dev_malloc((void**)&w->gp_ckpt, (ni * ram_gp_groups(w->capacity) + 1) * 4 * sizeof(u64)));
+    HIP_TRY(dev_malloc((void**)&w->gp_total, (n_blocks + 1) * 4 * sizeof(u64)));
     HIP_TRY(dev_malloc((void**)&w->nd_prefix, (ni * ram_nd_tiles(w->capacity) + 1) * sizeof(u32)));
     HIP_TRY(dev_malloc((void**)&w->instances, (ni + 1) * sizeof(zkw_ram_instance)));
     HIP_TRY(dev_malloc((void**)&w->nondet_counts, (ni + 1) * sizeof(u32)));
     HIP_TRY(dev_malloc((void**)&w->compact_forms, (ni + 1) * COMPACT_FORM_LEN * sizeof(u64)));
     HIP_TRY(dev_malloc((void**)&w->public_inputs, (ni + 1) * 4 * sizeof(u64)));
     return ZKW_OK;
-}
-
-__device__ __forceinline__ u32 block_of_position(const u64* __restrict__ offsets, int n_blocks, size_t i) {
-    int lo = 0, hi = n_blocks;
-    while (hi - lo > 1) {
-        int mid = (lo + hi) >> 1;
-        if (offsets[mid] <= i) lo = mid; else hi = mid;
-    }
-    return (u32)lo;
 }
 
 static __device__ __forceinline__ void k_ram_key_ranges(const VB& vb, const zkw_mem_query* __restrict__ q, size_t n, u32* __restrict__ maxima) {
@@ -1052,35 +1039,23 @@
     }
 }
 
-static __device__ __forceinline__ void k_ram_packed_keys(const VB& vb, const zkw_mem_query* __restrict__ q, size_t n, const u64* __restrict__ offsets,
-                                  int n_blocks, unsigned bits_p, unsigned bits_i, unsigned bits_t,
+static __device__ __forceinline__ void k_ram_packed_keys(const VB& vb, const zkw_mem_query* __restrict__ q, size_t n, unsigned bits_i, unsigned bits_t,
                                   u64* __restrict__ key, u32* __restrict__ iota) {
     size_t i = (size_t)vb.x * blockDim.x + threadIdx.x;
     if (i >= n) return;
-    u64 k = n_blocks > 1 ? block_of_position(offsets, n_blocks, i) : 0;
-    k = (k << bits_p) | q[i].page;
+    u64 k = q[i].page;
     k = (k << bits_i) | q[i].index;
     k = (k << bits_t) | q[i].timestamp;
     key[i] = k;
     iota[i] = (u32)i;
 }
 
-static __device__ __forceinline__ void k_ram_packed_cells(const VB& vb, const u64* __restrict__ cell, const u32* __restrict__ perm, size_t n,
-                                   const u64* __restrict__ offsets, int n_blocks, unsigned bits_p, unsigned bits_i,
+static __device__ __forceinline__ void k_ram_packed_cells(const VB& vb, const u64* __restrict__ cell, const u32* __restrict__ perm, size_t n, unsigned bits_i,
                                    u64* __restrict__ key) {
     size_t i = (size_t)vb.x * blockDim.x + threadIdx.x;
     if (i >= n) return;
-    const u32 src = perm[i];
-    const u64 c = cell[src];
-    u64 k = n_blocks > 1 ? block_of_position(offsets, n_blocks, src) : 0;
-    k = (k << bits_p) | (c >> 32);
-    k = (k << bits_i) | (c & 0xFFFFFFFFu);
-    key[i] = k;
-}
-
-static __device__ __forceinline__ void k_block_ids(const VB& vb, const u64* __restrict__ offsets, int n_blocks, size_t n, u32* __restrict__ ids) {
-    size_t i = (size_t)vb.x * blockDim.x + threadIdx.x;
-    if (i < n) ids[i] = block_of_position(offsets, n_blocks, i);
+    const u64 c = cell[perm[i]];
+    key[i] = ((c >> 32) << bits_i) | (c & 0xFFFFFFFFu);
 }
 
 static unsigned bits_in_use(u32 x) { return x ? 32u - (unsigned)__builtin_clz(x) : 0u; }
@@ -1088,7 +1063,7 @@
 static int ram_sort(zkw_ctx* ctx, const zkw_mem_query* d_q, size_t total, const std::vector<uint64_t>& offsets,
                     void* work_a, void* work_b, u32** perm_out) {
     const size_t n_blocks = offsets.size() - 1;
-    size_t tmp_bytes = radix_temp_bytes(total);
+    size_t tmp_bytes = radix_temp_bytes(total, n_blocks);
     u32* ts = static_cast<u32*>(work_a);
     u32 *k32 = ts + total, *v0 = k32 + total, *v1 = v0 + total;
     u64* cell = reinterpret_cast<u64*>(v1 + total);
@@ -1111,42 +1086,33 @@
     u32 maxima[4];
     ZKW_TRY(ctx->read_small(maxima, d_max, 16));
     const unsigned bits_t = bits_in_use(maxima[0]), bits_p = bits_in_use(maxima[1]), bits_i = bits_in_use(maxima[2]);
-    unsigned bits_b = 0;
-    while ((1ull << bits_b) < n_blocks) bits_b++;
-    u64* d_off = nullptr;
-    if (n_blocks > 1) ZKW_TRY(ctx->upload("sort_off", offsets, &d_off));
-
-    if (bits_b + bits_p + bits_i + bits_t <= 64) {
-        const unsigned bits = bits_b + bits_p + bits_i + bits_t;
-        { Prof _p(ctx, "k_ram_packed_keys");
-          ZKW_LAUNCH(ctx, k_ram_packed_keys, grid, 256, d_q, total, d_off, (int)n_blocks, bits_p, bits_i, bits_t, k64a, v0); }
+    std::vector<RsSeg> seg_table;
+    const u32 n_tiles = rs_seg_table(offsets.data(), n_blocks, seg_table), n_segs = (u32)n_blocks;
+    RsSeg* d_segs = nullptr;
+    ZKW_TRY(ctx->upload("sort_segs", seg_table, &d_segs));
+
+    if (bits_p + bits_i + bits_t <= 64) {
+        const unsigned bits = bits_p + bits_i + bits_t;
+        { Prof _p(ctx, "k_ram_packed_keys"); ZKW_LAUNCH(ctx, k_ram_packed_keys, grid, 256, d_q, total, bits_i, bits_t, k64a, v0); }
         ZKW_TRY(launch_check("k_ram_packed_keys"));
-        { Prof _p(ctx, "radix_sort"); ZKW_TRY(radix_sort_pairs<u64>(ctx, tmp, tmp_bytes, k64a, k64b, v0, v1, total, bits ? bits : 1)); }
+        { Prof _p(ctx, "radix_sort"); ZKW_TRY(radix_sort_pairs_segmented<u64>(ctx, tmp, tmp_bytes, k64a, k64b, v0, v1, total, d_segs, n_segs, n_tiles, bits)); }
         *perm_out = v1;
         return ZKW_OK;
     }
 
     { Prof _p(ctx, "k_ram_sort_keys"); ZKW_LAUNCH(ctx, k_ram_sort_keys, grid, 256, d_q, total, ts, cell, v0, (const u64*)nullptr, 0); }
     ZKW_TRY(launch_check("k_ram_sort_keys"));
-    { Prof _p(ctx, "radix_sort"); ZKW_TRY(radix_sort_pairs<u32>(ctx, tmp, tmp_bytes, ts, k32, v0, v1, total, bits_t ? bits_t : 1)); }
-    if (bits_b + bits_p + bits_i <= 64) {
-        const unsigned bits = bits_b + bits_p + bits_i;
-        { Prof _p(ctx, "k_ram_packed_cells");
-          ZKW_LAUNCH(ctx, k_ram_packed_cells, grid, 256, cell, v1, total, d_off, (int)n_blocks, bits_p, bits_i, k64a); }
+    { Prof _p(ctx, "radix_sort"); ZKW_TRY(radix_sort_pairs_segmented<u32>(ctx, tmp, tmp_bytes, ts, k32, v0, v1, total, d_segs, n_segs, n_tiles, bits_t)); }
+    const unsigned bits = bits_p + bits_i;
+    if (bits < 64) {
+        { Prof _p(ctx, "k_ram_packed_cells"); ZKW_LAUNCH(ctx, k_ram_packed_cells, grid, 256, cell, v1, total, bits_i, k64a); }
         ZKW_TRY(launch_check("k_ram_packed_cells"));
-        { Prof _p(ctx, "radix_sort"); ZKW_TRY(radix_sort_pairs<u64>(ctx, tmp, tmp_bytes, k64a, k64b, v1, v0, total, bits ? bits : 1)); }
-        *perm_out = v0;
-        return ZKW_OK;
-    }
-    { Prof _p(ctx, "k_gather_u64_by_u32"); ZKW_LAUNCH(ctx, k_gather_u64_by_u32, grid, 256, cell, v1, total, k64a); }
-    ZKW_TRY(launch_check("k_gather_u64_by_u32"));
-    { Prof _p(ctx, "radix_sort"); ZKW_TRY(radix_sort_pairs<u64>(ctx, tmp, tmp_bytes, k64a, k64b, v1, v0, total, 64)); }
-    { Prof _p(ctx, "k_block_ids"); ZKW_LAUNCH(ctx, k_block_ids, grid, 256, d_off, (int)n_blocks, total, ts); }
-    ZKW_TRY(launch_check("k_block_ids"));
-    { Prof _p(ctx, "k_gather_u32_by_u32"); ZKW_LAUNCH(ctx, k_gather_u32_by_u32, grid, 256, ts, v0, total, k32); }
-    ZKW_TRY(launch_check("k_gather_u32_by_u32"));
-    { Prof _p(ctx, "radix_sort"); ZKW_TRY(radix_sort_pairs<u32>(ctx, tmp, tmp_bytes, k32, ts, v0, v1, total, bits_b)); }
-    *perm_out = v1;
+    } else {
+        { Prof _p(ctx, "k_gather_u64_by_u32"); ZKW_LAUNCH(ctx, k_gather_u64_by_u32, grid, 256, cell, v1, total, k64a); }
+        ZKW_TRY(launch_check("k_gather_u64_by_u32"));
+    }
+    { Prof _p(ctx, "radix_sort"); ZKW_TRY(radix_sort_pairs_segmented<u64>(ctx, tmp, tmp_bytes, k64a, k64b, v1, v0, total, d_segs, n_segs, n_tiles, bits)); }
+    *perm_out = v0;
     return ZKW_OK;
 }
 
@@ -1195,40 +1161,40 @@
     }
     ZKW_TRY(dev_fs(ctx, fs, 12, 9));
     w->z_valid = false;
+    const size_t groups = ram_gp_groups(w->capacity), nd_tiles = ram_nd_tiles(w->capacity);
     for (size_t b0 = 0; b0 < n_blocks;) {
-        size_t b1 = b0 + 1;
-        while (b1 < n_blocks && w->offsets[b1 + 1] - w->offsets[b0] <= w->zcap) b1++;
-        ZKW_TRY(ram_gp_blocks(ctx, w, b0, b1, w->zbuf_l, w->zbuf_r));
-        const size_t base = w->offsets[b0];
+        const size_t b1 = std::min(n_blocks, b0 + 32768);
         std::vector<RamBlock> blocks(b1 - b0);
         size_t max_inst = 0;
         for (size_t b = b0; b < b1; b++) {
             const size_t lo = w->offsets[b], n = w->offsets[b + 1] - lo;
-            const size_t n_inst = w->inst_offsets[b + 1] - w->inst_offsets[b];
+            const size_t io = w->inst_offsets[b], n_inst = w->inst_offsets[b + 1] - io;
             if (n_inst > max_inst) max_inst = n_inst;
             blocks[b - b0] = RamBlock{w->unsorted_q,
                                       w->perm + lo,
-                                      w->unsorted_marks + 12 * w->inst_offsets[b],
-                                      w->sorted_marks + 12 * w->inst_offsets[b],
-                                      w->zbuf_l + 2 * (lo - base),
-                                      w->zbuf_r + 2 * (lo - base),
-                                      w->instances + w->inst_offsets[b],
-                                      w->nondet_counts + w->inst_offsets[b],
-                                      w->gp_ckpt + 4 * ram_gp_groups(w->capacity) * w->inst_offsets[b],
-                                      w->nd_prefix + ram_nd_tiles(w->capacity) * w->inst_offsets[b],
+                                      w->unsorted_q + lo,
+                                      w->challenges + 18 * b,
+                                      w->unsorted_marks + 12 * io,
+                                      w->sorted_marks + 12 * io,
+                                      w->instances + io,
+                                      w->nondet_counts + io,
+                                      w->gp_ckpt + 4 * groups * io,
+                                      w->gp_total + 4 * b,
+                                      w->nd_prefix + nd_tiles * io,
                                       n,
                                       w->capacity,
                                       n_nondet ? n_nondet[b] : 0u};
         }
         RamBlock* d_blocks = nullptr;
         ZKW_TRY(ctx->upload("ram_blocks", blocks, &d_blocks));
-        const unsigned gx = (unsigned)(max_inst < 64 ? max_inst : 64), gy = (unsigned)(b1 - b0);
-        { Prof _p(ctx, "k_ram_count_nondet"); ZKW_LAUNCH_2D(ctx, k_ram_count_nondet, gx, gy, 256, d_blocks); }
-        ZKW_TRY(launch_check("k_ram_count_nondet"));
+        const unsigned gy = (unsigned)(b1 - b0);
+        if (max_inst * nd_tiles >= (1ull << 31)) return fail(ZKW_ERR_INVALID, "ram_run: more than 2^31 - 1 tiles of 256 cycles in one block");
+        { Prof _p(ctx, "k_ram_gp_groups"); ZKW_LAUNCH_2D(ctx, k_ram_gp_groups, max_inst * nd_tiles, gy, 256, d_blocks); }
+        ZKW_TRY(launch_check("k_ram_gp_groups"));
+        { Prof _p(ctx, "k_ram_gp_scan"); ZKW_LAUNCH_2D(ctx, k_ram_gp_scan, 1, gy, 256, d_blocks); }
+        ZKW_TRY(launch_check("k_ram_gp_scan"));
         { Prof _p(ctx, "k_ram_instances"); ZKW_LAUNCH_2D(ctx, k_ram_instances, blocks_for(max_inst, 64), gy, 64, d_blocks); }
         ZKW_TRY(launch_check("k_ram_instances"));
-        { Prof _p(ctx, "k_ram_gp_ckpt"); ZKW_LAUNCH_2D(ctx, k_ram_gp_ckpt, blocks_for(max_inst * ram_gp_groups(w->capacity), 256), gy, 256, d_blocks); }
-        ZKW_TRY(launch_check("k_ram_gp_ckpt"));
         b0 = b1;
     }
     const size_t ni = w->n_instances;
```

New measurement: 3564, median of 6. +2.0%, better.
